# KKKSQJ/DeepLearning

Hardware: AMD Instinct MI355X
Metric: images/sec (higher is better)
Workload: dtype bf16; 1 GPU; model=resnet50, global_batch=256, image_size=224, parallelism=dp1

## Files before the change

### csrc/batchnorm.hip

```cpp
#include "common.h"
#include "vec.h"

namespace dla {

template <typename dev_t>
__global__ void bn_stats_kernel(const dev_t* __restrict__ x, float* __restrict__ sums,
                                int N, int C, int64_t HW) {
  __shared__ float smem[16];
  const int c = blockIdx.x;
  const int64_t total = (int64_t)N * HW;
  float sum = 0.f, sumsq = 0.f;
  for (int64_t m = (int64_t)blockIdx.y * blockDim.x + threadIdx.x; m < total;
       m += (int64_t)gridDim.y * blockDim.x) {
    const int64_t n = m / HW, hw = m % HW;
    const float f = to_f32(x[(n * C + c) * HW + hw]);
    sum += f;
    sumsq += f * f;
  }
  sum = block_reduce_sum(sum, smem);
  sumsq = block_reduce_sum(sumsq, smem);
  if (threadIdx.x == 0) {
    atomicAdd(&sums[c], sum);
    atomicAdd(&sums[C + c], sumsq);
  }
}

__device__ __forceinline__ void bn_finalize_channel(
    int c, float sum, float sumsq, const float* __restrict__ weight,
    const float* __restrict__ bias, float* __restrict__ mean,
    float* __restrict__ rstd, float* __restrict__ running_mean,
    float* __restrict__ running_var, float* __restrict__ scale,
    float* __restrict__ shift, float count, float eps, float momentum) {
  const float mu = sum / count;
  const float var = fmaxf(sumsq / count - mu * mu, 0.f);
  const float rs = rsqrtf(var + eps);
  mean[c] = mu;
  rstd[c] = rs;
  if (running_mean != nullptr && momentum > 0.f) {
    const float unbiased = var * count / fmaxf(count - 1.f, 1.f);
    running_mean[c] = (1.f - momentum) * running_mean[c] + momentum * mu;
    running_var[c] = (1.f - momentum) * running_var[c] + momentum * unbiased;
  }
  const float sc = weight[c] * rs;
  scale[c] = sc;
  shift[c] = bias[c] - mu * sc;
}

__global__ void bn_finalize_kernel(const float* __restrict__ sums,
                                   const float* __restrict__ weight,
                                   const float* __restrict__ bias,
                                   float* __restrict__ mean, float* __restrict__ rstd,
                                   float* __restrict__ running_mean,
                                   float* __restrict__ running_var,
                                   float* __restrict__ scale, float* __restrict__ shift,
                                   int C, float count, float eps, float momentum) {
  const int c = blockIdx.x * blockDim.x + threadIdx.x;
  if (c >= C) return;
  bn_finalize_channel(c, sums[c], sums[C + c], weight, bias, mean, rstd,
                      running_mean, running_var, scale, shift, count, eps,
                      momentum);
}

constexpr int kFinCh = 16, kFinRows = 64;

__global__ void __launch_bounds__(kFinCh * kFinRows)
bn_finalize_parts_kernel(const float* __restrict__ parts, int n_parts,
                         const float* __restrict__ weight,
                         const float* __restrict__ bias,
                         float* __restrict__ mean, float* __restrict__ rstd,
                         float* __restrict__ running_mean,
                         float* __restrict__ running_var,
                         float* __restrict__ scale, float* __restrict__ shift,
                         int C, float count, float eps, float momentum) {
  __shared__ float ls[2][kFinRows][kFinCh + 1];
  const int cl = threadIdx.x % kFinCh, rl = threadIdx.x / kFinCh;
  const int c = blockIdx.x * kFinCh + cl;
  float s = 0.f, q = 0.f;
  if (c < C) {
#pragma unroll 4
    for (int r = rl; r < n_parts; r += kFinRows) {
      const float* p = parts + (int64_t)r * 2 * C;
      s += p[c];
      q += p[C + c];
    }
  }
  ls[0][rl][cl] = s;
  ls[1][rl][cl] = q;
  __syncthreads();
  for (int h = kFinRows / 2; h > 0; h >>= 1) {
    if (rl < h) {
      ls[0][rl][cl] += ls[0][rl + h][cl];
      ls[1][rl][cl] += ls[1][rl + h][cl];
    }
    __syncthreads();
  }
  if (rl == 0 && c < C)
    bn_finalize_channel(c, ls[0][0][cl], ls[1][0][cl], weight, bias, mean,
                        rstd, running_mean, running_var, scale, shift, count,
                        eps, momentum);
}

template <typename dev_t, int V, bool RELU>
__global__ void bn_apply_kernel(const dev_t* __restrict__ x,
                                const float* __restrict__ scale,
                                const float* __restrict__ shift,
                                dev_t* __restrict__ y, int C, int64_t HW,
                                int64_t n_total) {
  const int64_t stride = (int64_t)gridDim.x * blockDim.x * V;
  for (int64_t i = ((int64_t)blockIdx.x * blockDim.x + threadIdx.x) * V;
       i < n_total; i += stride) {
    const int c = (int)((i / HW) % C);
    const float sc = scale[c], sh = shift[c];
    Vec<dev_t, V> xv = vload<dev_t, V>(x + i);
    Vec<dev_t, V> yv;
#pragma unroll
    for (int j = 0; j < V; ++j) {
      float f = to_f32(xv.v[j]) * sc + sh;
      yv.v[j] = from_f32<dev_t>(RELU ? fmaxf(f, 0.f) : f);
    }
    vstore<dev_t, V>(y + i, yv);
  }
}

template <typename dev_t, bool RELU>
__global__ void bn_bwd_stats_kernel(const dev_t* __restrict__ dy,
                                    const dev_t* __restrict__ x,
                                    const dev_t* __restrict__ y,
                                    const float* __restrict__ mean,
                                    const float* __restrict__ rstd,
                                    float* __restrict__ sums,
                                    int N, int C, int64_t HW) {
  __shared__ float smem[16];
  const int c = blockIdx.x;
  const float mu = mean[c], rs = rstd[c];
  const int64_t total = (int64_t)N * HW;
  float s_dy = 0.f, s_dyxh = 0.f;
  for (int64_t m = (int64_t)blockIdx.y * blockDim.x + threadIdx.x; m < total;
       m += (int64_t)gridDim.y * blockDim.x) {
    const int64_t n = m / HW, hw = m % HW;
    const int64_t idx = (n * C + c) * HW + hw;
    float g = to_f32(dy[idx]);
    if (RELU && to_f32(y[idx]) <= 0.f) g = 0.f;
    const float xh = (to_f32(x[idx]) - mu) * rs;
    s_dy += g;
    s_dyxh += g * xh;
  }
  s_dy = block_reduce_sum(s_dy, smem);
  s_dyxh = block_reduce_sum(s_dyxh, smem);
  if (threadIdx.x == 0) {
    atomicAdd(&sums[c], s_dy);
    atomicAdd(&sums[C + c], s_dyxh);
  }
}

template <typename dev_t, bool RELU>
__global__ void bn_bwd_dx_kernel(const dev_t* __restrict__ dy,
                                 const dev_t* __restrict__ x,
                                 const dev_t* __restrict__ y,
                                 const float* __restrict__ mean,
                                 const float* __restrict__ rstd,
                                 const float* __restrict__ weight,
                                 const float* __restrict__ sums,
                                 dev_t* __restrict__ dx, int C, int64_t HW,
                                 int64_t n_total, float inv_count) {
  const int64_t stride = (int64_t)gridDim.x * blockDim.x;
  for (int64_t i = (int64_t)blockIdx.x * blockDim.x + threadIdx.x; i < n_total;
       i += stride) {
    const int c = (int)((i / HW) % C);
    const float mu = mean[c], rs = rstd[c];
    float g = to_f32(dy[i]);
    if (RELU && to_f32(y[i]) <= 0.f) g = 0.f;
    const float xh = (to_f32(x[i]) - mu) * rs;
    const float m_dy = sums[c] * inv_count;
    const float m_dyxh = sums[C + c] * inv_count;
    dx[i] = from_f32<dev_t>(weight[c] * rs * (g - m_dy - xh * m_dyxh));
  }
}



inline int64_t nhwc_used_threads(int lanes_per_row, int64_t rows,
                                 int64_t target_lanes) {
  int64_t k = target_lanes / lanes_per_row;
  if (k > rows) k = rows;
  if (k < 1) k = 1;
  return (int64_t)lanes_per_row * k;
}

template <typename dev_t, int V>
__global__ void bn_stats_nhwc_kernel(const dev_t* __restrict__ x,
                                     float* __restrict__ sums, int C,
                                     int64_t rows, int64_t used) {
  extern __shared__ float ls[];
  for (int i = threadIdx.x; i < 2 * C; i += blockDim.x) ls[i] = 0.f;
  __syncthreads();
  const int64_t t = (int64_t)blockIdx.x * blockDim.x + threadIdx.x;
  const int lanes_per_row = C / V;
  if (t < used) {
    const int c0 = (int)(t % lanes_per_row) * V;
    const int64_t rstride = used / lanes_per_row;
    float s[V], q[V];
#pragma unroll
    for (int j = 0; j < V; ++j) { s[j] = 0.f; q[j] = 0.f; }
    for (int64_t r = t / lanes_per_row; r < rows; r += rstride) {
      Vec<dev_t, V> xv = vload<dev_t, V>(x + r * C + c0);
#pragma unroll
      for (int j = 0; j < V; ++j) {
        const float f = to_f32(xv.v[j]);
        s[j] += f;
        q[j] += f * f;
      }
    }
#pragma unroll
    for (int j = 0; j < V; ++j) {
      atomicAdd(&ls[c0 + j], s[j]);
      atomicAdd(&ls[C + c0 + j], q[j]);
    }
  }
  __syncthreads();
  for (int i = threadIdx.x; i < 2 * C; i += blockDim.x)
    atomicAdd(&sums[i], ls[i]);
}

template <typename dev_t, int V, bool RELU>
__global__ void bn_apply_nhwc_kernel(const dev_t* __restrict__ x,
                                     const float* __restrict__ scale,
                                     const float* __restrict__ shift,
                                     dev_t* __restrict__ y, int C, int64_t rows,
                                     int64_t used) {
  const int64_t t = (int64_t)blockIdx.x * blockDim.x + threadIdx.x;
  if (t >= used) return;
  const int lanes_per_row = C / V;
  const int c0 = (int)(t % lanes_per_row) * V;
  const int64_t rstride = used / lanes_per_row;
  float sc[V], sh[V];
#pragma unroll
  for (int j = 0; j < V; ++j) { sc[j] = scale[c0 + j]; sh[j] = shift[c0 + j]; }
  for (int64_t r = t / lanes_per_row; r < rows; r += rstride) {
    Vec<dev_t, V> xv = vload<dev_t, V>(x + r * C + c0);
    Vec<dev_t, V> yv;
#pragma unroll
    for (int j = 0; j < V; ++j) {
      const float f = to_f32(xv.v[j]) * sc[j] + sh[j];
      yv.v[j] = from_f32<dev_t>(RELU ? fmaxf(f, 0.f) : f);
    }
    vstore<dev_t, V>(y + r * C + c0, yv);
  }
}

template <typename dev_t, int V, bool RELU>
__global__ void bn_bwd_stats_nhwc_kernel(const dev_t* __restrict__ dy,
                                         const dev_t* __restrict__ x,
                                         const dev_t* __restrict__ y,
                                         const float* __restrict__ mean,
                                         const float* __restrict__ rstd,
                                         float* __restrict__ sums, int C,
                                         int64_t rows, int64_t used) {
  extern __shared__ float ls[];
  for (int i = threadIdx.x; i < 2 * C; i += blockDim.x) ls[i] = 0.f;
  __syncthreads();
  const int64_t t = (int64_t)blockIdx.x * blockDim.x + threadIdx.x;
  const int lanes_per_row = C / V;
  if (t < used) {
    const int c0 = (int)(t % lanes_per_row) * V;
    const int64_t rstride = used / lanes_per_row;
    float mu[V], rs[V], s_dy[V], s_dyxh[V];
#pragma unroll
    for (int j = 0; j < V; ++j) {
      mu[j] = mean[c0 + j];
      rs[j] = rstd[c0 + j];
      s_dy[j] = 0.f;
      s_dyxh[j] = 0.f;
    }
    for (int64_t r = t / lanes_per_row; r < rows; r += rstride) {
      const int64_t base = r * C + c0;
      Vec<dev_t, V> dyv = vload<dev_t, V>(dy + base);
      Vec<dev_t, V> xv = vload<dev_t, V>(x + base);
      Vec<dev_t, V> yv;
      if (RELU) yv = vload<dev_t, V>(y + base);
#pragma unroll
      for (int j = 0; j < V; ++j) {
        float g = to_f32(dyv.v[j]);
        if (RELU && to_f32(yv.v[j]) <= 0.f) g = 0.f;
        const float xh = (to_f32(xv.v[j]) - mu[j]) * rs[j];
        s_dy[j] += g;
        s_dyxh[j] += g * xh;
      }
    }
#pragma unroll
    for (int j = 0; j < V; ++j) {
      atomicAdd(&ls[c0 + j], s_dy[j]);
      atomicAdd(&ls[C + c0 + j], s_dyxh[j]);
    }
  }
  __syncthreads();
  for (int i = threadIdx.x; i < 2 * C; i += blockDim.x)
    atomicAdd(&sums[i], ls[i]);
}

template <typename dev_t, int V, bool RELU>
__global__ void bn_bwd_dx_nhwc_kernel(const dev_t* __restrict__ dy,
                                      const dev_t* __restrict__ x,
                                      const dev_t* __restrict__ y,
                                      const float* __restrict__ mean,
                                      const float* __restrict__ rstd,
                                      const float* __restrict__ weight,
                                      const float* __restrict__ sums,
                                      dev_t* __restrict__ dx, int C,
                                      int64_t rows, int64_t used,
                                      float inv_count) {
  const int64_t t = (int64_t)blockIdx.x * blockDim.x + threadIdx.x;
  if (t >= used) return;
  const int lanes_per_row = C / V;
  const int c0 = (int)(t % lanes_per_row) * V;
  const int64_t rstride = used / lanes_per_row;
  float mu[V], rs[V], wr[V], m_dy[V], m_dyxh[V];
#pragma unroll
  for (int j = 0; j < V; ++j) {
    mu[j] = mean[c0 + j];
    rs[j] = rstd[c0 + j];
    wr[j] = weight[c0 + j] * rs[j];
    m_dy[j] = sums[c0 + j] * inv_count;
    m_dyxh[j] = sums[C + c0 + j] * inv_count;
  }
  for (int64_t r = t / lanes_per_row; r < rows; r += rstride) {
    const int64_t base = r * C + c0;
    Vec<dev_t, V> dyv = vload<dev_t, V>(dy + base);
    Vec<dev_t, V> xv = vload<dev_t, V>(x + base);
    Vec<dev_t, V> yv;
    if (RELU) yv = vload<dev_t, V>(y + base);
    Vec<dev_t, V> dxv;
#pragma unroll
    for (int j = 0; j < V; ++j) {
      float g = to_f32(dyv.v[j]);
      if (RELU && to_f32(yv.v[j]) <= 0.f) g = 0.f;
      const float xh = (to_f32(xv.v[j]) - mu[j]) * rs[j];
      dxv.v[j] = from_f32<dev_t>(wr[j] * (g - m_dy[j] - xh * m_dyxh[j]));
    }
    vstore<dev_t, V>(dx + r * C + c0, dxv);
  }
}

template <typename dev_t, int V, bool DUAL>
__global__ void bn_add_relu_nhwc_kernel(const dev_t* __restrict__ x,
                                        const float* __restrict__ scale,
                                        const float* __restrict__ shift,
                                        const dev_t* __restrict__ idn,
                                        const float* __restrict__ scale_d,
                                        const float* __restrict__ shift_d,
                                        dev_t* __restrict__ out, int C,
                                        int64_t rows, int64_t used) {
  const int64_t t = (int64_t)blockIdx.x * blockDim.x + threadIdx.x;
  if (t >= used) return;
  const int lanes_per_row = C / V;
  const int c0 = (int)(t % lanes_per_row) * V;
  const int64_t rstride = used / lanes_per_row;
  float sc[V], sh[V], scd[V];
#pragma unroll
  for (int j = 0; j < V; ++j) {
    sc[j] = scale[c0 + j];
    sh[j] = shift[c0 + j];
    if (DUAL) {
      scd[j] = scale_d[c0 + j];
      sh[j] += shift_d[c0 + j];
    }
  }
  for (int64_t r = t / lanes_per_row; r < rows; r += rstride) {
    const int64_t base = r * C + c0;
    Vec<dev_t, V> xv = vload<dev_t, V>(x + base);
    Vec<dev_t, V> iv = vload<dev_t, V>(idn + base);
    Vec<dev_t, V> ov;
#pragma unroll
    for (int j = 0; j < V; ++j) {
      float f = to_f32(xv.v[j]) * sc[j] + sh[j];
      f += DUAL ? to_f32(iv.v[j]) * scd[j] : to_f32(iv.v[j]);
      ov.v[j] = from_f32<dev_t>(fmaxf(f, 0.f));
    }
    vstore<dev_t, V>(out + base, ov);
  }
}

template <typename dev_t, int V, bool DUAL>
__global__ void bn_join_bwd_stats_nhwc_kernel(
    const dev_t* __restrict__ dy, const dev_t* __restrict__ out,
    const dev_t* __restrict__ x, const float* __restrict__ mean,
    const float* __restrict__ rstd, const dev_t* __restrict__ xd,
    const float* __restrict__ mean_d, const float* __restrict__ rstd_d,
    dev_t* __restrict__ g_out, float* __restrict__ sums, int C, int64_t rows,
    int64_t used) {
  constexpr int NS = DUAL ? 3 : 2;
  extern __shared__ float ls[];
  for (int i = threadIdx.x; i < NS * C; i += blockDim.x) ls[i] = 0.f;
  __syncthreads();
  const int64_t t = (int64_t)blockIdx.x * blockDim.x + threadIdx.x;
  const int lanes_per_row = C / V;
  if (t < used) {
    const int c0 = (int)(t % lanes_per_row) * V;
    const int64_t rstride = used / lanes_per_row;
    float mu[V], rs[V], mud[V], rsd[V], s_g[V], s_gxh[V], s_gxhd[V];
#pragma unroll
    for (int j = 0; j < V; ++j) {
      mu[j] = mean[c0 + j];
      rs[j] = rstd[c0 + j];
      mud[j] = DUAL ? mean_d[c0 + j] : 0.f;
      rsd[j] = DUAL ? rstd_d[c0 + j] : 0.f;
      s_g[j] = 0.f;
      s_gxh[j] = 0.f;
      s_gxhd[j] = 0.f;
    }
    for (int64_t r = t / lanes_per_row; r < rows; r += rstride) {
      const int64_t base = r * C + c0;
      Vec<dev_t, V> dyv = vload<dev_t, V>(dy + base);
      Vec<dev_t, V> ov = vload<dev_t, V>(out + base);
      Vec<dev_t, V> xv = vload<dev_t, V>(x + base);
      Vec<dev_t, V> xdv;
      if (DUAL) xdv = vload<dev_t, V>(xd + base);
      Vec<dev_t, V> gv;
#pragma unroll
      for (int j = 0; j < V; ++j) {
        const bool on = to_f32(ov.v[j]) > 0.f;
        gv.v[j] = on ? dyv.v[j] : from_f32<dev_t>(0.f);
        const float g = on ? to_f32(dyv.v[j]) : 0.f;
        s_g[j] += g;
        s_gxh[j] += g * ((to_f32(xv.v[j]) - mu[j]) * rs[j]);
        if (DUAL) s_gxhd[j] += g * ((to_f32(xdv.v[j]) - mud[j]) * rsd[j]);
      }
      vstore<dev_t, V>(g_out + base, gv);
    }
#pragma unroll
    for (int j = 0; j < V; ++j) {
      atomicAdd(&ls[c0 + j], s_g[j]);
      atomicAdd(&ls[C + c0 + j], s_gxh[j]);
      if (DUAL) atomicAdd(&ls[2 * C + c0 + j], s_gxhd[j]);
    }
  }
  __syncthreads();
  for (int i = threadIdx.x; i < NS * C; i += blockDim.x)
    atomicAdd(&sums[i], ls[i]);
}

template <typename dev_t, int V>
__global__ void bn_join_bwd_dx_dual_nhwc_kernel(
    const dev_t* __restrict__ g, const dev_t* __restrict__ x,
    const dev_t* __restrict__ xd, const float* __restrict__ mean,
    const float* __restrict__ rstd, const float* __restrict__ weight,
    const float* __restrict__ mean_d, const float* __restrict__ rstd_d,
    const float* __restrict__ weight_d, const float* __restrict__ sums,
    dev_t* __restrict__ dx, dev_t* __restrict__ dxd, int C, int64_t rows,
    int64_t used, float inv_count) {
  const int64_t t = (int64_t)blockIdx.x * blockDim.x + threadIdx.x;
  if (t >= used) return;
  const int lanes_per_row = C / V;
  const int c0 = (int)(t % lanes_per_row) * V;
  const int64_t rstride = used / lanes_per_row;
  float mu[V], rs[V], wr[V], mud[V], rsd[V], wrd[V], m_g[V], m_gxh[V],
      m_gxhd[V];
#pragma unroll
  for (int j = 0; j < V; ++j) {
    mu[j] = mean[c0 + j];
    rs[j] = rstd[c0 + j];
    wr[j] = weight[c0 + j] * rs[j];
    mud[j] = mean_d[c0 + j];
    rsd[j] = rstd_d[c0 + j];
    wrd[j] = weight_d[c0 + j] * rsd[j];
    m_g[j] = sums[c0 + j] * inv_count;
    m_gxh[j] = sums[C + c0 + j] * inv_count;
    m_gxhd[j] = sums[2 * C + c0 + j] * inv_count;
  }
  for (int64_t r = t / lanes_per_row; r < rows; r += rstride) {
    const int64_t base = r * C + c0;
    Vec<dev_t, V> gv = vload<dev_t, V>(g + base);
    Vec<dev_t, V> xv = vload<dev_t, V>(x + base);
    Vec<dev_t, V> xdv = vload<dev_t, V>(xd + base);
    Vec<dev_t, V> dxv, dxdv;
#pragma unroll
    for (int j = 0; j < V; ++j) {
      const float gg = to_f32(gv.v[j]) - m_g[j];
      const float xh = (to_f32(xv.v[j]) - mu[j]) * rs[j];
      const float xhd = (to_f32(xdv.v[j]) - mud[j]) * rsd[j];
      dxv.v[j] = from_f32<dev_t>(wr[j] * (gg - xh * m_gxh[j]));
      dxdv.v[j] = from_f32<dev_t>(wrd[j] * (gg - xhd * m_gxhd[j]));
    }
    vstore<dev_t, V>(dx + base, dxv);
    vstore<dev_t, V>(dxd + base, dxdv);
  }
}

inline bool is_nhwc(const torch::Tensor& t) {
  return t.dim() == 4 && t.is_contiguous(at::MemoryFormat::ChannelsLast) &&
         !t.is_contiguous();
}

struct BnFinalized {
  torch::Tensor mean, rstd, scale, shift;
};

inline BnFinalized bn_finalize_launch(
    const torch::Tensor& sums, const torch::Tensor& weight,
    const torch::Tensor& bias, c10::optional<torch::Tensor>& running_mean,
    c10::optional<torch::Tensor>& running_var, int C, int64_t rows,
    double momentum, double eps) {
  TORCH_CHECK(sums.is_cuda() && sums.scalar_type() == torch::kFloat &&
                  sums.is_contiguous(),
              "bn sums must be a contiguous fp32 GPU tensor");
  TORCH_CHECK((sums.dim() == 1 && sums.size(0) == 2 * C) ||
                  (sums.dim() == 2 && sums.size(0) >= 1 &&
                   sums.size(1) == 2 * C),
              "bn sums must be [2C] or [n_parts, 2C]");
  TORCH_CHECK(weight.numel() == C && bias.numel() == C,
              "bn weight/bias must have C elements");
  auto opts_f = sums.options();
  BnFinalized f{torch::empty({C}, opts_f), torch::empty({C}, opts_f),
                torch::empty({C}, opts_f), torch::empty({C}, opts_f)};
  auto w32 = weight.to(torch::kFloat).contiguous();
  auto b32 = bias.to(torch::kFloat).contiguous();
  float* rm = running_mean.has_value() ? running_mean->data_ptr<float>() : nullptr;
  float* rv = running_var.has_value() ? running_var->data_ptr<float>() : nullptr;
  const int n_parts = sums.dim() == 2 ? (int)sums.size(0) : 1;
  if (n_parts > 1) {
    hipLaunchKernelGGL(bn_finalize_parts_kernel, dim3((C + kFinCh - 1) / kFinCh),
                       dim3(kFinCh * kFinRows), 0, stream(),
                       sums.data_ptr<float>(), n_parts, w32.data_ptr<float>(),
                       b32.data_ptr<float>(), f.mean.data_ptr<float>(),
                       f.rstd.data_ptr<float>(), rm, rv,
                       f.scale.data_ptr<float>(), f.shift.data_ptr<float>(), C,
                       (float)rows, (float)eps, (float)momentum);
  } else {
    hipLaunchKernelGGL(bn_finalize_kernel, dim3((C + 255) / 256), dim3(256), 0,
                       stream(), sums.data_ptr<float>(), w32.data_ptr<float>(),
                       b32.data_ptr<float>(), f.mean.data_ptr<float>(),
                       f.rstd.data_ptr<float>(), rm, rv,
                       f.scale.data_ptr<float>(), f.shift.data_ptr<float>(), C,
                       (float)rows, (float)eps, (float)momentum);
  }
  return f;
}

inline torch::Tensor bn_param_grad(const torch::Tensor& sums, int64_t offset,
                                   int C, const torch::Tensor& weight) {
  return sums.narrow(0, offset, C).to(weight.scalar_type());
}

inline bool is_nhwc_rows(const torch::Tensor& t) {
  return t.dim() == 4 && t.is_contiguous(at::MemoryFormat::ChannelsLast);
}

}

std::vector<torch::Tensor> batchnorm_fwd(torch::Tensor x, torch::Tensor weight,
                                         torch::Tensor bias,
                                         c10::optional<torch::Tensor> running_mean,
                                         c10::optional<torch::Tensor> running_var,
                                         double momentum, double eps, bool relu) {
  DLA_CHECK_CUDA(x);
  TORCH_CHECK(x.dim() == 4, "batchnorm_fwd expects a 4D tensor");
  const bool nhwc = dla::is_nhwc(x);
  TORCH_CHECK(nhwc || x.is_contiguous(), "batchnorm_fwd: x must be contiguous "
              "(NCHW or channels_last)");
  const int N = (int)x.size(0), C = (int)x.size(1);
  const int64_t HW = x.size(2) * x.size(3);
  auto opts_f = x.options().dtype(torch::kFloat);
  auto sums = torch::zeros({2 * C}, opts_f);
  auto mean = torch::empty({C}, opts_f);
  auto rstd = torch::empty({C}, opts_f);
  auto scale = torch::empty({C}, opts_f);
  auto shift = torch::empty({C}, opts_f);
  auto y = torch::empty_like(x);
  auto w32 = weight.to(torch::kFloat);
  auto b32 = bias.to(torch::kFloat);

  const int64_t rows = (int64_t)N * HW;
  const int ysplit = (int)std::min<int64_t>((rows + 65535) / 65536 + 1,
                                            std::max(1, 2048 / C));
  DLA_DISPATCH_FLOAT_TYPES(x.scalar_type(), "batchnorm_fwd", [&] {
    if (nhwc) {
      constexpr int VM = 16 / (int)sizeof(dev_t);
      auto stats = [&](auto vtag) {
        constexpr int V = decltype(vtag)::value;
        const int lanes = C / V;
        const int64_t used = dla::nhwc_used_threads(lanes, rows, 262144);
        const int lds = 2 * C * sizeof(float);
        hipLaunchKernelGGL((dla::bn_stats_nhwc_kernel<dev_t, V>),
                           dim3((int)((used + 255) / 256)), dim3(256), lds,
                           dla::stream(), (const dev_t*)x.data_ptr(),
                           sums.data_ptr<float>(), C, rows, used);
      };
      if (C % VM == 0) stats(std::integral_constant<int, VM>{});
      else if (C % 2 == 0) stats(std::integral_constant<int, 2>{});
      else stats(std::integral_constant<int, 1>{});
    } else {
      hipLaunchKernelGGL((dla::bn_stats_kernel<dev_t>), dim3(C, ysplit), dim3(256), 0,
                         dla::stream(), (const dev_t*)x.data_ptr(),
                         sums.data_ptr<float>(), N, C, HW);
    }
    hipLaunchKernelGGL(dla::bn_finalize_kernel, dim3((C + 255) / 256), dim3(256), 0,
                       dla::stream(), sums.data_ptr<float>(), w32.data_ptr<float>(),
                       b32.data_ptr<float>(), mean.data_ptr<float>(),
                       rstd.data_ptr<float>(),
                       running_mean.has_value() ? running_mean->data_ptr<float>() : nullptr,
                       running_var.has_value() ? running_var->data_ptr<float>() : nullptr,
                       scale.data_ptr<float>(), shift.data_ptr<float>(), C,
                       (float)rows, (float)eps, (float)momentum);
    const int64_t n_total = x.numel();
    constexpr int VMAX = 16 / (int)sizeof(dev_t);
    auto launch = [&](auto vtag, auto rtag) {
      constexpr int V = decltype(vtag)::value;
      constexpr bool R = decltype(rtag)::value;
      if (nhwc) {
        const int lanes = C / V;
        const int64_t used = dla::nhwc_used_threads(lanes, rows, 524288);
        hipLaunchKernelGGL((dla::bn_apply_nhwc_kernel<dev_t, V, R>),
                           dim3((int)((used + 255) / 256)), dim3(256), 0,
                           dla::stream(), (const dev_t*)x.data_ptr(),
                           scale.data_ptr<float>(), shift.data_ptr<float>(),
                           (dev_t*)y.data_ptr(), C, rows, used);
        return;
      }
      const int grid = dla::grid_1d((n_total + V - 1) / V, 256);
      if (false) ;
      else
        hipLaunchKernelGGL((dla::bn_apply_kernel<dev_t, V, R>), dim3(grid), dim3(256),
                           0, dla::stream(), (const dev_t*)x.data_ptr(),
                           scale.data_ptr<float>(), shift.data_ptr<float>(),
                           (dev_t*)y.data_ptr(), C, HW, n_total);
    };
    const bool vec_ok = nhwc ? (C % VMAX == 0) : (HW % VMAX == 0);
    if (vec_ok) {
      if (relu) launch(std::integral_constant<int, VMAX>{}, std::true_type{});
      else launch(std::integral_constant<int, VMAX>{}, std::false_type{});
    } else {
      if (relu) launch(std::integral_constant<int, 1>{}, std::true_type{});
      else launch(std::integral_constant<int, 1>{}, std::false_type{});
    }
  });
  HIP_CHECK_ERR();
  return {y, mean, rstd};
}

std::vector<torch::Tensor> batchnorm_fwd_from_sums(
    torch::Tensor x, torch::Tensor weight, torch::Tensor bias,
    torch::Tensor sums, c10::optional<torch::Tensor> running_mean,
    c10::optional<torch::Tensor> running_var, double momentum, double eps,
    bool relu) {
  DLA_CHECK_CUDA(x);
  TORCH_CHECK(x.dim() == 4, "batchnorm_fwd_from_sums expects a 4D tensor");
  const bool nhwc = dla::is_nhwc(x);
  TORCH_CHECK(nhwc || x.is_contiguous(),
              "batchnorm_fwd_from_sums: x must be contiguous");
  const int N = (int)x.size(0), C = (int)x.size(1);
  const int64_t HW = x.size(2) * x.size(3);
  auto y = torch::empty_like(x);
  const int64_t rows = (int64_t)N * HW;
  auto fin = dla::bn_finalize_launch(sums, weight, bias, running_mean,
                                     running_var, C, rows, momentum, eps);
  auto& mean = fin.mean;
  auto& rstd = fin.rstd;
  auto& scale = fin.scale;
  auto& shift = fin.shift;
  DLA_DISPATCH_FLOAT_TYPES(x.scalar_type(), "batchnorm_fwd_from_sums", [&] {
    const int64_t n_total = x.numel();
    constexpr int VMAX = 16 / (int)sizeof(dev_t);
    auto launch = [&](auto vtag, auto rtag) {
      constexpr int V = decltype(vtag)::value;
      constexpr bool R = decltype(rtag)::value;
      if (nhwc) {
        const int lanes = C / V;
        const int64_t used = dla::nhwc_used_threads(lanes, rows, 524288);
        hipLaunchKernelGGL((dla::bn_apply_nhwc_kernel<dev_t, V, R>),
                           dim3((int)((used + 255) / 256)), dim3(256), 0,
                           dla::stream(), (const dev_t*)x.data_ptr(),
                           scale.data_ptr<float>(), shift.data_ptr<float>(),
                           (dev_t*)y.data_ptr(), C, rows, used);
        return;
      }
      const int grid = dla::grid_1d((n_total + V - 1) / V, 256);
      hipLaunchKernelGGL((dla::bn_apply_kernel<dev_t, V, R>), dim3(grid),
                         dim3(256), 0, dla::stream(),
                         (const dev_t*)x.data_ptr(), scale.data_ptr<float>(),
                         shift.data_ptr<float>(), (dev_t*)y.data_ptr(), C, HW,
                         n_total);
    };
    const bool vec_ok = nhwc ? (C % VMAX == 0) : (HW % VMAX == 0);
    if (vec_ok) {
      if (relu) launch(std::integral_constant<int, VMAX>{}, std::true_type{});
      else launch(std::integral_constant<int, VMAX>{}, std::false_type{});
    } else {
      if (relu) launch(std::integral_constant<int, 1>{}, std::true_type{});
      else launch(std::integral_constant<int, 1>{}, std::false_type{});
    }
  });
  HIP_CHECK_ERR();
  return {y, mean, rstd};
}

torch::Tensor bn_apply(torch::Tensor x, torch::Tensor scale, torch::Tensor shift,
                       bool relu) {
  DLA_CHECK_CUDA(x);
  TORCH_CHECK(x.dim() == 4, "bn_apply expects a 4D tensor");
  const bool nhwc = dla::is_nhwc(x);
  TORCH_CHECK(nhwc || x.is_contiguous(), "bn_apply: x must be contiguous");
  const int C = (int)x.size(1);
  const int64_t HW = x.size(2) * x.size(3);
  auto y = torch::empty_like(x);
  auto sc = scale.to(torch::kFloat).contiguous();
  auto sh = shift.to(torch::kFloat).contiguous();
  const int64_t n_total = x.numel();
  DLA_DISPATCH_FLOAT_TYPES(x.scalar_type(), "bn_apply", [&] {
    constexpr int VMAX = 16 / (int)sizeof(dev_t);
    auto launch = [&](auto vtag, auto rtag) {
      constexpr int V = decltype(vtag)::value;
      constexpr bool R = decltype(rtag)::value;
      if (nhwc) {
        const int64_t rows = n_total / C;
        const int lanes = C / V;
        const int64_t used = dla::nhwc_used_threads(lanes, rows, 524288);
        hipLaunchKernelGGL((dla::bn_apply_nhwc_kernel<dev_t, V, R>),
                           dim3((int)((used + 255) / 256)), dim3(256), 0,
                           dla::stream(), (const dev_t*)x.data_ptr(),
                           sc.data_ptr<float>(), sh.data_ptr<float>(),
                           (dev_t*)y.data_ptr(), C, rows, used);
        return;
      }
      const int grid = dla::grid_1d((n_total + V - 1) / V, 256);
      if (false) ;
      else
        hipLaunchKernelGGL((dla::bn_apply_kernel<dev_t, V, R>), dim3(grid), dim3(256),
                           0, dla::stream(), (const dev_t*)x.data_ptr(),
                           sc.data_ptr<float>(), sh.data_ptr<float>(),
                           (dev_t*)y.data_ptr(), C, HW, n_total);
    };
    const bool vec_ok = nhwc ? (C % VMAX == 0) : (HW % VMAX == 0);
    if (vec_ok) {
      if (relu) launch(std::integral_constant<int, VMAX>{}, std::true_type{});
      else launch(std::integral_constant<int, VMAX>{}, std::false_type{});
    } else {
      if (relu) launch(std::integral_constant<int, 1>{}, std::true_type{});
      else launch(std::integral_constant<int, 1>{}, std::false_type{});
    }
  });
  HIP_CHECK_ERR();
  return y;
}

std::vector<torch::Tensor> batchnorm_bwd(torch::Tensor dy, torch::Tensor x,
                                         c10::optional<torch::Tensor> y,
                                         torch::Tensor weight, torch::Tensor mean,
                                         torch::Tensor rstd, bool relu) {
  DLA_CHECK_CUDA(dy); DLA_CHECK_CUDA(x);
  const bool nhwc = dla::is_nhwc(x);
  TORCH_CHECK(nhwc || x.is_contiguous(), "batchnorm_bwd: x must be contiguous");
  if (nhwc && !dla::is_nhwc(dy)) dy = dy.contiguous(at::MemoryFormat::ChannelsLast);
  if (!nhwc) dy = dy.contiguous();
  const int N = (int)x.size(0), C = (int)x.size(1);
  const int64_t HW = x.size(2) * x.size(3);
  const int64_t rows = (int64_t)N * HW;
  auto opts_f = x.options().dtype(torch::kFloat);
  auto sums = torch::zeros({2 * C}, opts_f);
  auto dx = torch::empty_like(x);
  auto w32 = weight.to(torch::kFloat);
  const int ysplit = (int)std::min<int64_t>((rows + 65535) / 65536 + 1,
                                            std::max(1, 2048 / C));
  TORCH_CHECK(!relu || y.has_value(), "batchnorm_bwd: relu mask needs y");
  DLA_DISPATCH_FLOAT_TYPES(x.scalar_type(), "batchnorm_bwd", [&] {
    const dev_t* yp = y.has_value() ? (const dev_t*)y->data_ptr() : nullptr;
    auto launch_stats = [&](auto rtag) {
      constexpr bool R = decltype(rtag)::value;
      if (nhwc) {
        constexpr int VM = 16 / (int)sizeof(dev_t);
        auto stats = [&](auto vtag) {
          constexpr int V = decltype(vtag)::value;
          const int lanes = C / V;
          const int64_t used = dla::nhwc_used_threads(lanes, rows, 262144);
          const int lds = 2 * C * sizeof(float);
          hipLaunchKernelGGL((dla::bn_bwd_stats_nhwc_kernel<dev_t, V, R>),
                             dim3((int)((used + 255) / 256)), dim3(256), lds,
                             dla::stream(), (const dev_t*)dy.data_ptr(),
                             (const dev_t*)x.data_ptr(), yp, mean.data_ptr<float>(),
                             rstd.data_ptr<float>(), sums.data_ptr<float>(), C,
                             rows, used);
        };
        if (C % VM == 0) stats(std::integral_constant<int, VM>{});
        else if (C % 2 == 0) stats(std::integral_constant<int, 2>{});
        else stats(std::integral_constant<int, 1>{});
      } else {
        hipLaunchKernelGGL((dla::bn_bwd_stats_kernel<dev_t, R>), dim3(C, ysplit),
                           dim3(256), 0, dla::stream(), (const dev_t*)dy.data_ptr(),
                           (const dev_t*)x.data_ptr(), yp, mean.data_ptr<float>(),
                           rstd.data_ptr<float>(), sums.data_ptr<float>(), N, C, HW);
      }
    };
    if (relu) launch_stats(std::true_type{});
    else launch_stats(std::false_type{});

    const int64_t n_total = x.numel();
    const float inv_count = 1.f / (float)rows;
    constexpr int VMAX = 16 / (int)sizeof(dev_t);
    auto launch_dx = [&](auto vtag, auto rtag) {
      constexpr int V = decltype(vtag)::value;
      constexpr bool R = decltype(rtag)::value;
      if (nhwc) {
        const int lanes = C / V;
        const int64_t used = dla::nhwc_used_threads(lanes, rows, 524288);
        hipLaunchKernelGGL((dla::bn_bwd_dx_nhwc_kernel<dev_t, V, R>),
                           dim3((int)((used + 255) / 256)), dim3(256), 0,
                           dla::stream(), (const dev_t*)dy.data_ptr(),
                           (const dev_t*)x.data_ptr(), yp, mean.data_ptr<float>(),
                           rstd.data_ptr<float>(), w32.data_ptr<float>(),
                           sums.data_ptr<float>(), (dev_t*)dx.data_ptr(), C,
                           rows, used, inv_count);
      } else {
        hipLaunchKernelGGL((dla::bn_bwd_dx_kernel<dev_t, R>), dim3(dla::grid_1d(n_total, 256)),
                           dim3(256), 0, dla::stream(), (const dev_t*)dy.data_ptr(),
                           (const dev_t*)x.data_ptr(), yp, mean.data_ptr<float>(),
                           rstd.data_ptr<float>(), w32.data_ptr<float>(),
                           sums.data_ptr<float>(), (dev_t*)dx.data_ptr(), C, HW,
                           n_total, inv_count);
      }
    };
    const bool vec_ok = nhwc && (C % VMAX == 0);
    if (vec_ok) {
      if (relu) launch_dx(std::integral_constant<int, VMAX>{}, std::true_type{});
      else launch_dx(std::integral_constant<int, VMAX>{}, std::false_type{});
    } else {
      if (relu) launch_dx(std::integral_constant<int, 1>{}, std::true_type{});
      else launch_dx(std::integral_constant<int, 1>{}, std::false_type{});
    }
  });
  HIP_CHECK_ERR();
  return {dx, dla::bn_param_grad(sums, C, C, weight),
          dla::bn_param_grad(sums, 0, C, weight)};
}

namespace dla {

inline void join_check(const torch::Tensor& x, const torch::Tensor& other,
                       const char* what) {
  TORCH_CHECK(other.is_cuda() && other.scalar_type() == x.scalar_type() &&
                  other.sizes() == x.sizes() && is_nhwc_rows(other),
              "bn join: ", what, " must match x (shape, dtype, channels_last)");
}

inline int join_vec(const torch::Tensor& x) {
  const int vmax = 16 / (int)x.element_size();
  TORCH_CHECK(x.size(1) % vmax == 0,
              "bn join: C must be a multiple of ", vmax);
  return vmax;
}

}

std::vector<torch::Tensor> bn_add_relu_fwd_from_sums(
    torch::Tensor x, torch::Tensor weight, torch::Tensor bias,
    torch::Tensor sums, c10::optional<torch::Tensor> running_mean,
    c10::optional<torch::Tensor> running_var, double momentum, double eps,
    torch::Tensor identity) {
  DLA_CHECK_CUDA(x);
  TORCH_CHECK(dla::is_nhwc_rows(x), "bn_add_relu: x must be channels_last");
  dla::join_check(x, identity, "identity");
  dla::join_vec(x);
  const int C = (int)x.size(1);
  const int64_t rows = x.numel() / C;
  auto fin = dla::bn_finalize_launch(sums, weight, bias, running_mean,
                                     running_var, C, rows, momentum, eps);
  auto out = torch::empty_like(x);
  DLA_DISPATCH_FLOAT_TYPES(x.scalar_type(), "bn_add_relu_fwd_from_sums", [&] {
    constexpr int V = 16 / (int)sizeof(dev_t);
    const int64_t used = dla::nhwc_used_threads(C / V, rows, 524288);
    hipLaunchKernelGGL((dla::bn_add_relu_nhwc_kernel<dev_t, V, false>),
                       dim3((int)((used + 255) / 256)), dim3(256), 0,
                       dla::stream(), (const dev_t*)x.data_ptr(),
                       fin.scale.data_ptr<float>(), fin.shift.data_ptr<float>(),
                       (const dev_t*)identity.data_ptr(), nullptr, nullptr,
                       (dev_t*)out.data_ptr(), C, rows, used);
  });
  HIP_CHECK_ERR();
  return {out, fin.mean, fin.rstd};
}

std::vector<torch::Tensor> bn_add_relu_dual_fwd_from_sums(
    torch::Tensor x, torch::Tensor weight, torch::Tensor bias,
    torch::Tensor sums, c10::optional<torch::Tensor> running_mean,
    c10::optional<torch::Tensor> running_var, double momentum, double eps,
    torch::Tensor xd, torch::Tensor weight_d, torch::Tensor bias_d,
    torch::Tensor sums_d, c10::optional<torch::Tensor> running_mean_d,
    c10::optional<torch::Tensor> running_var_d, double momentum_d,
    double eps_d) {
  DLA_CHECK_CUDA(x);
  TORCH_CHECK(dla::is_nhwc_rows(x), "bn_add_relu_dual: x must be channels_last");
  dla::join_check(x, xd, "xd");
  dla::join_vec(x);
  const int C = (int)x.size(1);
  const int64_t rows = x.numel() / C;
  auto fin = dla::bn_finalize_launch(sums, weight, bias, running_mean,
                                     running_var, C, rows, momentum, eps);
  auto fd = dla::bn_finalize_launch(sums_d, weight_d, bias_d, running_mean_d,
                                    running_var_d, C, rows, momentum_d, eps_d);
  auto out = torch::empty_like(x);
  DLA_DISPATCH_FLOAT_TYPES(x.scalar_type(), "bn_add_relu_dual_fwd_from_sums", [&] {
    constexpr int V = 16 / (int)sizeof(dev_t);
    const int64_t used = dla::nhwc_used_threads(C / V, rows, 524288);
    hipLaunchKernelGGL((dla::bn_add_relu_nhwc_kernel<dev_t, V, true>),
                       dim3((int)((used + 255) / 256)), dim3(256), 0,
                       dla::stream(), (const dev_t*)x.data_ptr(),
                       fin.scale.data_ptr<float>(), fin.shift.data_ptr<float>(),
                       (const dev_t*)xd.data_ptr(), fd.scale.data_ptr<float>(),
                       fd.shift.data_ptr<float>(), (dev_t*)out.data_ptr(), C,
                       rows, used);
  });
  HIP_CHECK_ERR();
  return {out, fin.mean, fin.rstd, fd.mean, fd.rstd};
}

std::vector<torch::Tensor> bn_add_relu_bwd(torch::Tensor dy, torch::Tensor out,
                                           torch::Tensor x, torch::Tensor weight,
                                           torch::Tensor mean,
                                           torch::Tensor rstd) {
  DLA_CHECK_CUDA(x);
  TORCH_CHECK(dla::is_nhwc_rows(x), "bn_add_relu_bwd: x must be channels_last");
  dla::join_check(x, out, "out");
  if (!dla::is_nhwc_rows(dy)) dy = dy.contiguous(at::MemoryFormat::ChannelsLast);
  dla::join_check(x, dy, "dy");
  dla::join_vec(x);
  const int C = (int)x.size(1);
  const int64_t rows = x.numel() / C;
  TORCH_CHECK(mean.numel() == C && rstd.numel() == C && weight.numel() == C,
              "bn_add_relu_bwd: per-channel tensors must have C elements");
  auto sums = torch::zeros({2 * C}, x.options().dtype(torch::kFloat));
  auto g = torch::empty_like(x);
  auto dx = torch::empty_like(x);
  auto w32 = weight.to(torch::kFloat).contiguous();
  DLA_DISPATCH_FLOAT_TYPES(x.scalar_type(), "bn_add_relu_bwd", [&] {
    constexpr int V = 16 / (int)sizeof(dev_t);
    const int lanes = C / V;
    const int64_t used_s = dla::nhwc_used_threads(lanes, rows, 262144);
    hipLaunchKernelGGL((dla::bn_join_bwd_stats_nhwc_kernel<dev_t, V, false>),
                       dim3((int)((used_s + 255) / 256)), dim3(256),
                       2 * C * sizeof(float), dla::stream(),
                       (const dev_t*)dy.data_ptr(), (const dev_t*)out.data_ptr(),
                       (const dev_t*)x.data_ptr(), mean.data_ptr<float>(),
                       rstd.data_ptr<float>(), nullptr, nullptr, nullptr,
                       (dev_t*)g.data_ptr(), sums.data_ptr<float>(), C, rows,
                       used_s);
    const int64_t used = dla::nhwc_used_threads(lanes, rows, 524288);
    hipLaunchKernelGGL((dla::bn_bwd_dx_nhwc_kernel<dev_t, V, false>),
                       dim3((int)((used + 255) / 256)), dim3(256), 0,
                       dla::stream(), (const dev_t*)g.data_ptr(),
                       (const dev_t*)x.data_ptr(), nullptr,
                       mean.data_ptr<float>(), rstd.data_ptr<float>(),
                       w32.data_ptr<float>(), sums.data_ptr<float>(),
                       (dev_t*)dx.data_ptr(), C, rows, used,
                       1.f / (float)rows);
  });
  HIP_CHECK_ERR();
  return {g, dx, dla::bn_param_grad(sums, C, C, weight),
          dla::bn_param_grad(sums, 0, C, weight)};
}

std::vector<torch::Tensor> bn_add_relu_dual_bwd(
    torch::Tensor dy, torch::Tensor out, torch::Tensor x, torch::Tensor weight,
    torch::Tensor mean, torch::Tensor rstd, torch::Tensor xd,
    torch::Tensor weight_d, torch::Tensor mean_d, torch::Tensor rstd_d) {
  DLA_CHECK_CUDA(x);
  TORCH_CHECK(dla::is_nhwc_rows(x), "bn_add_relu_dual_bwd: x must be channels_last");
  dla::join_check(x, out, "out");
  dla::join_check(x, xd, "xd");
  if (!dla::is_nhwc_rows(dy)) dy = dy.contiguous(at::MemoryFormat::ChannelsLast);
  dla::join_check(x, dy, "dy");
  dla::join_vec(x);
  const int C = (int)x.size(1);
  const int64_t rows = x.numel() / C;
  TORCH_CHECK(mean.numel() == C && rstd.numel() == C && weight.numel() == C &&
                  mean_d.numel() == C && rstd_d.numel() == C &&
                  weight_d.numel() == C,
              "bn_add_relu_dual_bwd: per-channel tensors must have C elements");
  auto sums = torch::zeros({3 * C}, x.options().dtype(torch::kFloat));
  auto g = torch::empty_like(x);
  auto dx = torch::empty_like(x);
  auto dxd = torch::empty_like(x);
  auto w32 = weight.to(torch::kFloat).contiguous();
  auto wd32 = weight_d.to(torch::kFloat).contiguous();
  DLA_DISPATCH_FLOAT_TYPES(x.scalar_type(), "bn_add_relu_dual_bwd", [&] {
    constexpr int V = 16 / (int)sizeof(dev_t);
    const int lanes = C / V;
    const int64_t used_s = dla::nhwc_used_threads(lanes, rows, 262144);
    hipLaunchKernelGGL((dla::bn_join_bwd_stats_nhwc_kernel<dev_t, V, true>),
                       dim3((int)((used_s + 255) / 256)), dim3(256),
                       3 * C * sizeof(float), dla::stream(),
                       (const dev_t*)dy.data_ptr(), (const dev_t*)out.data_ptr(),
                       (const dev_t*)x.data_ptr(), mean.data_ptr<float>(),
                       rstd.data_ptr<float>(), (const dev_t*)xd.data_ptr(),
                       mean_d.data_ptr<float>(), rstd_d.data_ptr<float>(),
                       (dev_t*)g.data_ptr(), sums.data_ptr<float>(), C, rows,
                       used_s);
    const int64_t used = dla::nhwc_used_threads(lanes, rows, 524288);
    hipLaunchKernelGGL((dla::bn_join_bwd_dx_dual_nhwc_kernel<dev_t, V>),
                       dim3((int)((used + 255) / 256)), dim3(256), 0,
                       dla::stream(), (const dev_t*)g.data_ptr(),
                       (const dev_t*)x.data_ptr(), (const dev_t*)xd.data_ptr(),
                       mean.data_ptr<float>(), rstd.data_ptr<float>(),
                       w32.data_ptr<float>(), mean_d.data_ptr<float>(),
                       rstd_d.data_ptr<float>(), wd32.data_ptr<float>(),
                       sums.data_ptr<float>(), (dev_t*)dx.data_ptr(),
                       (dev_t*)dxd.data_ptr(), C, rows, used,
                       1.f / (float)rows);
  });
  HIP_CHECK_ERR();
  auto dbias = dla::bn_param_grad(sums, 0, C, weight);
  return {dx, dxd, dla::bn_param_grad(sums, C, C, weight), dbias,
          dla::bn_param_grad(sums, 2 * C, C, weight_d),
          dbias.to(weight_d.scalar_type()).clone()};
}
```

### csrc/bindings.cpp

```cpp
#include <torch/extension.h>

std::vector<torch::Tensor> layernorm_fwd(torch::Tensor x, torch::Tensor w,
                                         torch::Tensor b, double eps);
std::vector<torch::Tensor> layernorm_bwd(torch::Tensor dy, torch::Tensor x,
                                         torch::Tensor w, torch::Tensor mean,
                                         torch::Tensor rstd);
torch::Tensor gelu_fwd(torch::Tensor x);
torch::Tensor gelu_bwd(torch::Tensor dy, torch::Tensor x);
torch::Tensor silu_fwd(torch::Tensor x);
torch::Tensor silu_bwd(torch::Tensor dy, torch::Tensor x);
torch::Tensor add_relu_fwd(torch::Tensor a, torch::Tensor b);
torch::Tensor relu_mask_bwd(torch::Tensor dy, torch::Tensor y);
std::vector<torch::Tensor> batchnorm_fwd(torch::Tensor x, torch::Tensor weight,
                                         torch::Tensor bias,
                                         c10::optional<torch::Tensor> running_mean,
                                         c10::optional<torch::Tensor> running_var,
                                         double momentum, double eps, bool relu);
torch::Tensor bn_apply(torch::Tensor x, torch::Tensor scale, torch::Tensor shift,
                       bool relu);
std::vector<torch::Tensor> batchnorm_bwd(torch::Tensor dy, torch::Tensor x,
                                         c10::optional<torch::Tensor> y,
                                         torch::Tensor weight, torch::Tensor mean,
                                         torch::Tensor rstd, bool relu);
std::vector<torch::Tensor> batchnorm_fwd_from_sums(
    torch::Tensor x, torch::Tensor weight, torch::Tensor bias,
    torch::Tensor sums, c10::optional<torch::Tensor> running_mean,
    c10::optional<torch::Tensor> running_var, double momentum, double eps,
    bool relu);
std::vector<torch::Tensor> bn_add_relu_fwd_from_sums(
    torch::Tensor x, torch::Tensor weight, torch::Tensor bias,
    torch::Tensor sums, c10::optional<torch::Tensor> running_mean,
    c10::optional<torch::Tensor> running_var, double momentum, double eps,
    torch::Tensor identity);
std::vector<torch::Tensor> bn_add_relu_dual_fwd_from_sums(
    torch::Tensor x, torch::Tensor weight, torch::Tensor bias,
    torch::Tensor sums, c10::optional<torch::Tensor> running_mean,
    c10::optional<torch::Tensor> running_var, double momentum, double eps,
    torch::Tensor xd, torch::Tensor weight_d, torch::Tensor bias_d,
    torch::Tensor sums_d, c10::optional<torch::Tensor> running_mean_d,
    c10::optional<torch::Tensor> running_var_d, double momentum_d,
    double eps_d);
std::vector<torch::Tensor> bn_add_relu_bwd(torch::Tensor dy, torch::Tensor out,
                                           torch::Tensor x, torch::Tensor weight,
                                           torch::Tensor mean,
                                           torch::Tensor rstd);
std::vector<torch::Tensor> bn_add_relu_dual_bwd(
    torch::Tensor dy, torch::Tensor out, torch::Tensor x, torch::Tensor weight,
    torch::Tensor mean, torch::Tensor rstd, torch::Tensor xd,
    torch::Tensor weight_d, torch::Tensor mean_d, torch::Tensor rstd_d);
std::vector<torch::Tensor> conv1x1_fwd(torch::Tensor a, torch::Tensor b,
                                       c10::optional<torch::Tensor> bias,
                                       c10::optional<torch::Tensor> scale,
                                       c10::optional<torch::Tensor> shift,
                                       c10::optional<torch::Tensor> residual,
                                       bool relu, bool want_stats);
torch::Tensor conv1x1_wgrad(torch::Tensor dy, torch::Tensor x);
std::vector<torch::Tensor> conv3x3_fwd(torch::Tensor a, torch::Tensor w9,
                                       int64_t imgH, int64_t imgW,
                                       c10::optional<torch::Tensor> bias,
                                       c10::optional<torch::Tensor> scale,
                                       c10::optional<torch::Tensor> shift,
                                       c10::optional<torch::Tensor> residual,
                                       bool relu, bool want_stats);
torch::Tensor conv3x3_wgrad(torch::Tensor dy, torch::Tensor x, int64_t imgH,
                            int64_t imgW);
torch::Tensor transpose2d(torch::Tensor src);
torch::Tensor stride2_gather(torch::Tensor x);
torch::Tensor stride2_scatter(torch::Tensor dy, int64_t IH, int64_t IW);
std::vector<torch::Tensor> softmax_ce_fwd(torch::Tensor logits,
                                          c10::optional<torch::Tensor> target,
                                          c10::optional<torch::Tensor> soft_target,
                                          double smoothing, int64_t ignore_index);
torch::Tensor softmax_ce_bwd(torch::Tensor logits,
                             c10::optional<torch::Tensor> target,
                             c10::optional<torch::Tensor> soft_target,
                             torch::Tensor lse, double smoothing,
                             int64_t ignore_index, torch::Tensor grad_out,
                             torch::Tensor stats);
torch::Tensor focal_loss_fwd(torch::Tensor logits, torch::Tensor targets,
                             double alpha, double gamma);
torch::Tensor focal_loss_bwd(torch::Tensor dloss, torch::Tensor logits,
                             torch::Tensor targets, double alpha, double gamma);
torch::Tensor box_iou_gpu(torch::Tensor a, torch::Tensor b, bool giou);
torch::Tensor nms_gpu(torch::Tensor boxes_sorted, double iou_threshold);
torch::Tensor roialign_fwd(torch::Tensor input, torch::Tensor rois, int64_t PH,
                           int64_t PW, double spatial_scale,
                           int64_t sampling_ratio, bool aligned);
torch::Tensor roialign_bwd(torch::Tensor grad_out, torch::Tensor rois, int64_t N,
                           int64_t C, int64_t H, int64_t W, double spatial_scale,
                           int64_t sampling_ratio, bool aligned);
std::vector<torch::Tensor> attn_fwd(torch::Tensor qkv, int64_t num_heads,
                                    double scale,
                                    c10::optional<torch::Tensor> bias,
                                    c10::optional<torch::Tensor> mask,
                                    bool save_p, bool save_stats);
std::vector<torch::Tensor> attn_bwd(torch::Tensor qkv, torch::Tensor dout,
                                    torch::Tensor stats, torch::Tensor drow,
                                    int64_t num_heads, double scale);
std::vector<torch::Tensor> attn_fwd_cosine(torch::Tensor qkv, int64_t num_heads,
                              torch::Tensor logit_scale,
                              c10::optional<torch::Tensor> bias,
                              c10::optional<torch::Tensor> mask, bool save_p);
torch::Tensor mfma_probe(torch::Tensor A, torch::Tensor B);
torch::Tensor my_add(torch::Tensor a, torch::Tensor b);
std::vector<torch::Tensor> cocoeval_match_image(
    torch::Tensor det_boxes, torch::Tensor det_scores, torch::Tensor gt_boxes,
    torch::Tensor gt_crowd, torch::Tensor iou_thrs, int64_t max_dets,
    c10::optional<torch::Tensor> gt_extra_ignore);
torch::Tensor window_partition_fwd(torch::Tensor x, int64_t ws, int64_t shift);
torch::Tensor window_partition_bwd(torch::Tensor grad, int64_t B, int64_t H,
                                   int64_t W, int64_t ws, int64_t shift);
torch::Tensor window_merge_fwd(torch::Tensor windows, int64_t B, int64_t H,
                               int64_t W, int64_t ws, int64_t shift);
torch::Tensor window_merge_bwd(torch::Tensor grad, int64_t ws, int64_t shift);

PYBIND11_MODULE(TORCH_EXTENSION_NAME, m) {
  m.doc() = "deeplearning_amd gfx950 HIP kernels";
  m.def("layernorm_fwd", &layernorm_fwd);
  m.def("layernorm_bwd", &layernorm_bwd);
  m.def("gelu_fwd", &gelu_fwd);
  m.def("gelu_bwd", &gelu_bwd);
  m.def("silu_fwd", &silu_fwd);
  m.def("silu_bwd", &silu_bwd);
  m.def("add_relu_fwd", &add_relu_fwd);
  m.def("relu_mask_bwd", &relu_mask_bwd);
  m.def("batchnorm_fwd", &batchnorm_fwd);
  m.def("batchnorm_fwd_from_sums", &batchnorm_fwd_from_sums);
  m.def("bn_apply", &bn_apply);
  m.def("batchnorm_bwd", &batchnorm_bwd);
  m.def("bn_add_relu_fwd_from_sums", &bn_add_relu_fwd_from_sums);
  m.def("bn_add_relu_dual_fwd_from_sums", &bn_add_relu_dual_fwd_from_sums);
  m.def("bn_add_relu_bwd", &bn_add_relu_bwd);
  m.def("bn_add_relu_dual_bwd", &bn_add_relu_dual_bwd);
  m.def("conv1x1_fwd", &conv1x1_fwd, py::arg("a"), py::arg("b"),
        py::arg("bias") = py::none(), py::arg("scale") = py::none(),
        py::arg("shift") = py::none(), py::arg("residual") = py::none(),
        py::arg("relu") = false, py::arg("want_stats") = false);
  m.def("conv1x1_wgrad", &conv1x1_wgrad);
  m.def("conv3x3_fwd", &conv3x3_fwd, py::arg("a"), py::arg("w9"),
        py::arg("imgH"), py::arg("imgW"), py::arg("bias") = py::none(),
        py::arg("scale") = py::none(), py::arg("shift") = py::none(),
        py::arg("residual") = py::none(), py::arg("relu") = false,
        py::arg("want_stats") = false);
  m.def("conv3x3_wgrad", &conv3x3_wgrad);
  m.def("transpose2d", &transpose2d);
  m.def("stride2_gather", &stride2_gather);
  m.def("stride2_scatter", &stride2_scatter);
  m.def("softmax_ce_fwd", &softmax_ce_fwd);
  m.def("softmax_ce_bwd", &softmax_ce_bwd);
  m.def("focal_loss_fwd", &focal_loss_fwd);
  m.def("focal_loss_bwd", &focal_loss_bwd);
  m.def("box_iou", &box_iou_gpu);
  m.def("nms", &nms_gpu);
  m.def("roialign_fwd", &roialign_fwd);
  m.def("roialign_bwd", &roialign_bwd);
  m.def("attn_fwd", &attn_fwd, py::arg("qkv"), py::arg("num_heads"),
        py::arg("scale"), py::arg("bias") = py::none(),
        py::arg("mask") = py::none(), py::arg("save_p") = false,
        py::arg("save_stats") = false);
  m.def("attn_bwd", &attn_bwd);
  m.def("attn_fwd_cosine", &attn_fwd_cosine, py::arg("qkv"),
        py::arg("num_heads"), py::arg("logit_scale"),
        py::arg("bias") = py::none(), py::arg("mask") = py::none(),
        py::arg("save_p") = false);
  m.def("mfma_probe", &mfma_probe);
  m.def("cocoeval_match_image", &cocoeval_match_image, py::arg("det_boxes"),
        py::arg("det_scores"), py::arg("gt_boxes"), py::arg("gt_crowd"),
        py::arg("iou_thrs"), py::arg("max_dets"),
        py::arg("gt_extra_ignore") = py::none());
  m.def("my_add", &my_add);
  m.def("window_partition_fwd", &window_partition_fwd);
  m.def("window_partition_bwd", &window_partition_bwd);
  m.def("window_merge_fwd", &window_merge_fwd);
  m.def("window_merge_bwd", &window_merge_bwd);
}
```

### deeplearning_amd/models/classification/resnet.py

```python
from __future__ import annotations

import torch
import torch.nn as nn

from ...ops import BatchNorm2d, add_relu
from ...ops.conv1x1 import (can_pass_input, conv1x1_bn, conv_bn,
                            conv_bn_add_relu)
from ..registry import register_model


def _downsample_fwd(downsample, x):
    if (isinstance(downsample, nn.Sequential) and len(downsample) == 2 and
            isinstance(downsample[0], nn.Conv2d)):
        return conv_bn(x, downsample[0], downsample[1])
    return downsample(x)


class _NormRelu(nn.Sequential):

    def __init__(self, norm, c):
        super().__init__(norm(c), nn.ReLU(inplace=True))


def make_norm(norm_layer, c, relu=False):
    if not relu:
        return norm_layer(c)
    try:
        return norm_layer(c, relu=True)
    except TypeError:
        return _NormRelu(norm_layer, c)


def conv3x3(cin, cout, stride=1, groups=1, dilation=1):
    return nn.Conv2d(cin, cout, 3, stride=stride, padding=dilation, groups=groups,
                     bias=False, dilation=dilation)


def conv1x1(cin, cout, stride=1):
    return nn.Conv2d(cin, cout, 1, stride=stride, bias=False)


class BasicBlock(nn.Module):
    expansion = 1

    def __init__(self, inplanes, planes, stride=1, downsample=None, groups=1,
                 base_width=64, dilation=1, norm_layer=None):
        super().__init__()
        norm_layer = norm_layer or BatchNorm2d
        if groups != 1 or base_width != 64:
            raise ValueError("BasicBlock only supports groups=1, base_width=64")
        self.conv1 = conv3x3(inplanes, planes, stride)
        self.bn1 = make_norm(norm_layer, planes, relu=True)
        self.conv2 = conv3x3(planes, planes)
        self.bn2 = norm_layer(planes)
        self.downsample = downsample
        self.stride = stride

    def forward(self, x):
        identity = x
        out = conv_bn(x, self.conv1, self.bn1)
        out = conv_bn(out, self.conv2, self.bn2)
        if self.downsample is not None:
            identity = _downsample_fwd(self.downsample, x)
        return add_relu(out, identity)


class Bottleneck(nn.Module):
    expansion = 4

    def __init__(self, inplanes, planes, stride=1, downsample=None, groups=1,
                 base_width=64, dilation=1, norm_layer=None):
        super().__init__()
        norm_layer = norm_layer or BatchNorm2d
        width = int(planes * (base_width / 64.0)) * groups
        self.conv1 = conv1x1(inplanes, width)
        self.bn1 = make_norm(norm_layer, width, relu=True)
        self.conv2 = conv3x3(width, width, stride, groups, dilation)
        self.bn2 = make_norm(norm_layer, width, relu=True)
        self.conv3 = conv1x1(width, planes * self.expansion)
        self.bn3 = norm_layer(planes * self.expansion)
        self.downsample = downsample
        self.stride = stride

    def forward(self, x):
        identity = x
        if self.downsample is None and can_pass_input(x, self.conv1, self.bn1):
            out, identity = conv1x1_bn(x, self.conv1, self.bn1,
                                       pass_input=True)
        else:
            out = conv_bn(x, self.conv1, self.bn1)
        out = conv_bn(out, self.conv2, self.bn2)
        return conv_bn_add_relu(out, self.conv3, self.bn3, identity=identity,
                                x_down=x, downsample=self.downsample)


class ResNet(nn.Module):
    def __init__(self, block, layers, num_classes=1000, groups=1, width_per_group=64,
                 replace_stride_with_dilation=None, norm_layer=None,
                 zero_init_residual=False, include_top=True):
        super().__init__()
        self._norm_layer = norm_layer or BatchNorm2d
        self.inplanes = 64
        self.dilation = 1
        replace_stride_with_dilation = replace_stride_with_dilation or [False] * 3
        self.groups = groups
        self.base_width = width_per_group
        self.include_top = include_top

        self.conv1 = nn.Conv2d(3, 64, 7, stride=2, padding=3, bias=False)
        self.bn1 = make_norm(self._norm_layer, 64, relu=True)
        self.maxpool = nn.MaxPool2d(3, stride=2, padding=1)
        self.layer1 = self._make_layer(block, 64, layers[0])
        self.layer2 = self._make_layer(block, 128, layers[1], stride=2,
                                       dilate=replace_stride_with_dilation[0])
        self.layer3 = self._make_layer(block, 256, layers[2], stride=2,
                                       dilate=replace_stride_with_dilation[1])
        self.layer4 = self._make_layer(block, 512, layers[3], stride=2,
                                       dilate=replace_stride_with_dilation[2])
        if include_top:
            self.avgpool = nn.AdaptiveAvgPool2d(1)
            self.fc = nn.Linear(512 * block.expansion, num_classes)

        for m in self.modules():
            if isinstance(m, nn.Conv2d):
                nn.init.kaiming_normal_(m.weight, mode="fan_out", nonlinearity="relu")
            elif isinstance(m, (nn.BatchNorm2d, nn.GroupNorm)):
                nn.init.ones_(m.weight)
                nn.init.zeros_(m.bias)
        if zero_init_residual:
            for m in self.modules():
                if isinstance(m, Bottleneck):
                    nn.init.zeros_(m.bn3.weight)
                elif isinstance(m, BasicBlock):
                    nn.init.zeros_(m.bn2.weight)

    def _make_layer(self, block, planes, blocks, stride=1, dilate=False):
        norm_layer = self._norm_layer
        downsample = None
        prev_dilation = self.dilation
        if dilate:
            self.dilation *= stride
            stride = 1
        if stride != 1 or self.inplanes != planes * block.expansion:
            downsample = nn.Sequential(
                conv1x1(self.inplanes, planes * block.expansion, stride),
                norm_layer(planes * block.expansion),
            )
        layers = [block(self.inplanes, planes, stride, downsample, self.groups,
                        self.base_width, prev_dilation, norm_layer)]
        self.inplanes = planes * block.expansion
        for _ in range(1, blocks):
            layers.append(block(self.inplanes, planes, groups=self.groups,
                                base_width=self.base_width, dilation=self.dilation,
                                norm_layer=norm_layer))
        return nn.Sequential(*layers)

    def forward_features(self, x):
        x = self.maxpool(self.bn1(self.conv1(x)))
        x = self.layer1(x)
        x = self.layer2(x)
        x = self.layer3(x)
        x = self.layer4(x)
        return x

    def forward(self, x):
        x = self.forward_features(x)
        if self.include_top:
            x = self.avgpool(x)
            x = torch.flatten(x, 1)
            x = self.fc(x)
        return x


@register_model
def resnet18(num_classes=1000, **kw):
    return ResNet(BasicBlock, [2, 2, 2, 2], num_classes=num_classes, **kw)


@register_model
def resnet34(num_classes=1000, **kw):
    return ResNet(BasicBlock, [3, 4, 6, 3], num_classes=num_classes, **kw)


@register_model
def resnet50(num_classes=1000, **kw):
    return ResNet(Bottleneck, [3, 4, 6, 3], num_classes=num_classes, **kw)


@register_model
def resnet101(num_classes=1000, **kw):
    return ResNet(Bottleneck, [3, 4, 23, 3], num_classes=num_classes, **kw)


@register_model
def resnet152(num_classes=1000, **kw):
    return ResNet(Bottleneck, [3, 8, 36, 3], num_classes=num_classes, **kw)


@register_model
def resnext50_32x4d(num_classes=1000, **kw):
    return ResNet(Bottleneck, [3, 4, 6, 3], num_classes=num_classes, groups=32,
                  width_per_group=4, **kw)


@register_model
def resnext101_32x8d(num_classes=1000, **kw):
    return ResNet(Bottleneck, [3, 4, 23, 3], num_classes=num_classes, groups=32,
                  width_per_group=8, **kw)


@register_model
def wide_resnet50_2(num_classes=1000, **kw):
    return ResNet(Bottleneck, [3, 4, 6, 3], num_classes=num_classes,
                  width_per_group=128, **kw)


@register_model
def wide_resnet101_2(num_classes=1000, **kw):
    return ResNet(Bottleneck, [3, 4, 23, 3], num_classes=num_classes,
                  width_per_group=128, **kw)
```

### deeplearning_amd/ops/__init__.py

```python
from ._ext import ext, has_ext, use_hip
from .activations import GELU, SiLU, add_relu, gelu, silu
from .batchnorm import BatchNorm2d, FrozenBatchNorm2d
from .conv1x1 import conv1x1_bn, conv_bn, conv_bn_add_relu
from .boxes import (batched_nms, bbox_iou_aligned, box_area, box_iou,
                    clip_boxes_to_image, generalized_box_iou, nms,
                    remove_small_boxes)
from .drop import DropPath, drop_path
from .ema import ModelEMA
from .layernorm import LayerNorm, LayerNorm2d, layer_norm
from .losses import (CrossEntropyLoss, cross_entropy, sigmoid_focal_loss,
                     soft_target_cross_entropy)
from .roi_align import MultiScaleRoIAlign, roi_align
from .window import (roll_and_window_partition, window_merge_and_roll,
                     window_partition_eager, window_reverse_eager)

__all__ = [
    "ext", "has_ext", "use_hip",
    "gelu", "silu", "add_relu", "GELU", "SiLU",
    "BatchNorm2d", "FrozenBatchNorm2d",
    "conv_bn", "conv1x1_bn", "conv_bn_add_relu",
    "box_iou", "generalized_box_iou", "bbox_iou_aligned", "box_area", "nms",
    "batched_nms", "clip_boxes_to_image", "remove_small_boxes",
    "DropPath", "drop_path", "ModelEMA",
    "LayerNorm", "LayerNorm2d", "layer_norm",
    "CrossEntropyLoss", "cross_entropy", "soft_target_cross_entropy",
    "sigmoid_focal_loss",
    "MultiScaleRoIAlign", "roi_align",
    "roll_and_window_partition", "window_merge_and_roll",
    "window_partition_eager", "window_reverse_eager",
]
```

### deeplearning_amd/ops/batchnorm.py

```python
from __future__ import annotations

import torch
import torch.nn as nn
import torch.nn.functional as F

from ._ext import dense, ext, use_hip


class _BNFn(torch.autograd.Function):
    @staticmethod
    def forward(ctx, x, weight, bias, running_mean, running_var, momentum, eps, relu):
        x = dense(x)
        y, mean, rstd = ext().batchnorm_fwd(
            x, weight, bias, running_mean, running_var, momentum, eps, relu)
        ctx.save_for_backward(x, y, weight, mean, rstd)
        ctx.relu = relu
        return y

    @staticmethod
    def backward(ctx, dy):
        x, y, weight, mean, rstd = ctx.saved_tensors
        dx, dw, db = ext().batchnorm_bwd(
            dy, x, y if ctx.relu else None, weight, mean, rstd, ctx.relu)
        return dx, dw, db, None, None, None, None, None


class BatchNorm2d(nn.BatchNorm2d):

    def __init__(self, num_features, eps=1e-5, momentum=0.1, relu=False):
        super().__init__(num_features, eps=eps, momentum=momentum, affine=True,
                         track_running_stats=True)
        self.relu = relu

    def _eaf(self) -> float:
        if self.momentum is not None:
            return self.momentum
        if self.training and self.num_batches_tracked is not None:
            return 1.0 / float(max(int(self.num_batches_tracked), 1))
        return 0.0

    def forward(self, x):
        if not use_hip(x):
            if self.training and self.momentum is None and \
                    self.num_batches_tracked is not None:
                self.num_batches_tracked.add_(1)
            y = F.batch_norm(x, self.running_mean, self.running_var, self.weight,
                             self.bias, self.training, self._eaf(), self.eps)
            return torch.relu(y) if self.relu else y
        if self.running_mean.dtype != torch.float32:
            self.running_mean.data = self.running_mean.data.float()
            self.running_var.data = self.running_var.data.float()
        if self.training:
            if self.num_batches_tracked is not None:
                self.num_batches_tracked.add_(1)
            return _BNFn.apply(x, self.weight, self.bias, self.running_mean,
                               self.running_var, self._eaf(), self.eps,
                               self.relu)
        rstd = torch.rsqrt(self.running_var.float() + self.eps)
        scale = self.weight.float() * rstd
        shift = self.bias.float() - self.running_mean.float() * scale
        if torch.is_grad_enabled() and (x.requires_grad or self.weight.requires_grad):
            y = x * scale.reshape(1, -1, 1, 1).to(x.dtype) + shift.reshape(1, -1, 1, 1).to(x.dtype)
            return torch.relu(y) if self.relu else y
        return ext().bn_apply(dense(x), scale, shift, self.relu)


class FrozenBatchNorm2d(nn.Module):

    def __init__(self, num_features, eps=1e-5):
        super().__init__()
        self.eps = eps
        self.register_buffer("weight", torch.ones(num_features))
        self.register_buffer("bias", torch.zeros(num_features))
        self.register_buffer("running_mean", torch.zeros(num_features))
        self.register_buffer("running_var", torch.ones(num_features))

    def _load_from_state_dict(self, state_dict, prefix, *args, **kwargs):
        state_dict.pop(prefix + "num_batches_tracked", None)
        super()._load_from_state_dict(state_dict, prefix, *args, **kwargs)

    def forward(self, x):
        rstd = torch.rsqrt(self.running_var.float() + self.eps)
        scale = self.weight.float() * rstd
        shift = self.bias.float() - self.running_mean.float() * scale
        if use_hip(x) and not (torch.is_grad_enabled() and x.requires_grad):
            return ext().bn_apply(dense(x), scale, shift, False)
        sc = scale.reshape(1, -1, 1, 1).to(x.dtype)
        sh = shift.reshape(1, -1, 1, 1).to(x.dtype)
        return x * sc + sh
```

### deeplearning_amd/ops/conv1x1.py

```python
from __future__ import annotations

import os

import torch
import torch.nn.functional as F
from torch import nn

from ._ext import ext, use_hip


def _flatten_nhwc(x: torch.Tensor) -> torch.Tensor:
    B, C, H, W = x.shape
    return x.permute(0, 2, 3, 1).reshape(B * H * W, C)


def _unflatten_nhwc(y2d: torch.Tensor, B: int, H: int, W: int) -> torch.Tensor:
    return y2d.view(B, H, W, -1).permute(0, 3, 1, 2)


class _Conv1x1Fn(torch.autograd.Function):

    @staticmethod
    def forward(ctx, x2d, w, bias, scale, shift, residual, relu, want_stats,
                pass_input=False):
        xb = x2d if x2d.dtype == torch.bfloat16 else x2d.to(torch.bfloat16)
        wb = w if w.dtype == torch.bfloat16 else w.to(torch.bfloat16)
        wb = wb.contiguous()
        y2d, sums = ext().conv1x1_fwd(xb, wb, bias, scale, shift, residual,
                                      relu, want_stats)
        ctx.save_for_backward(xb, wb)
        ctx.x_dtype = x2d.dtype
        ctx.w_dtype = w.dtype
        ctx.pass_input = pass_input
        outs = (y2d,)
        if want_stats:
            ctx.mark_non_differentiable(sums)
            outs += (sums,)
        if pass_input:
            ctx.set_materialize_grads(False)
            outs += (x2d,)
        return outs if len(outs) > 1 else y2d

    @staticmethod
    def backward(ctx, dy2d, *rest):
        xb, wb = ctx.saved_tensors
        d_alias = rest[-1] if ctx.pass_input else None
        if d_alias is not None:
            d_alias = d_alias.contiguous()
        dx = dw = db = None
        if dy2d is None:
            if d_alias is not None and ctx.needs_input_grad[0]:
                dx = d_alias.to(ctx.x_dtype)
            return dx, None, None, None, None, None, None, None, None
        dy2d = dy2d.contiguous()
        if dy2d.dtype != torch.bfloat16:
            dy2d = dy2d.to(torch.bfloat16)
        if ctx.needs_input_grad[0]:
            wt = ext().transpose2d(wb)
            if d_alias is not None and d_alias.dtype != torch.bfloat16:
                d_alias = d_alias.to(torch.bfloat16)
            dx, _ = ext().conv1x1_fwd(dy2d, wt, None, None, None, d_alias,
                                      False, False)
            if dx.dtype != ctx.x_dtype:
                dx = dx.to(ctx.x_dtype)
        if ctx.needs_input_grad[1]:
            dw = ext().conv1x1_wgrad(dy2d, xb)
            if dw.dtype != ctx.w_dtype:
                dw = dw.to(ctx.w_dtype)
        if ctx.needs_input_grad[2]:
            db = dy2d.float().sum(0)
        return dx, dw, db, None, None, None, None, None, None


class _BNFromStatsFn(torch.autograd.Function):

    @staticmethod
    def forward(ctx, x, weight, bias, sums, running_mean, running_var,
                momentum, eps, relu):
        y, mean, rstd = ext().batchnorm_fwd_from_sums(
            x, weight, bias, sums, running_mean, running_var, momentum, eps,
            relu)
        ctx.save_for_backward(x, y, weight, mean, rstd)
        ctx.relu = relu
        return y

    @staticmethod
    def backward(ctx, dy):
        x, y, weight, mean, rstd = ctx.saved_tensors
        dx, dw, db = ext().batchnorm_bwd(
            dy, x, y if ctx.relu else None, weight, mean, rstd, ctx.relu)
        return dx, dw, db, None, None, None, None, None, None


class _Stride2Fn(torch.autograd.Function):

    @staticmethod
    def forward(ctx, x):
        ctx.ihw = (x.shape[2], x.shape[3])
        return ext().stride2_gather(x)

    @staticmethod
    def backward(ctx, dy):
        if not dy.is_contiguous(memory_format=torch.channels_last):
            dy = dy.contiguous(memory_format=torch.channels_last)
        return ext().stride2_scatter(dy, *ctx.ihw)


def _conv1x1_disabled() -> bool:
    return os.environ.get("DLA_NO_CONV1X1", "0") == "1"


def can_fuse_conv1x1(x: torch.Tensor, conv: nn.Conv2d) -> bool:
    if _conv1x1_disabled() or not use_hip(x):
        return False
    if x.dtype != torch.bfloat16:
        return False
    if conv.kernel_size != (1, 1) or conv.groups != 1:
        return False
    if conv.padding != (0, 0) or conv.dilation != (1, 1):
        return False
    if conv.stride not in ((1, 1), (2, 2)):
        return False
    cin, cout = conv.in_channels, conv.out_channels
    if cin % 64 != 0 or cout % 64 != 0:
        return False
    return x.dim() == 4 and x.is_contiguous(memory_format=torch.channels_last)


def _prep(x: torch.Tensor, conv: nn.Conv2d):
    stride = conv.stride[0]
    if stride == 2:
        x = _Stride2Fn.apply(x)
    B, C, H, W = x.shape
    x2d = _flatten_nhwc(x)
    w2d = conv.weight.reshape(conv.weight.shape[0], conv.weight.shape[1])
    bias = conv.bias.float() if conv.bias is not None else None
    return x2d, w2d, bias, (B, H, W)


def conv1x1(x: torch.Tensor, conv: nn.Conv2d) -> torch.Tensor:
    x2d, wb, bias, (B, H, W) = _prep(x, conv)
    y2d = _Conv1x1Fn.apply(x2d, wb, bias, None, None, None, False, False)
    return _unflatten_nhwc(y2d, B, H, W)


def _fp32_running_stats(bn) -> None:
    if bn.running_mean.dtype != torch.float32:
        bn.running_mean.data = bn.running_mean.data.float()
        bn.running_var.data = bn.running_var.data.float()


def _conv1x1_train_stats(x: torch.Tensor, conv: nn.Conv2d, bn,
                         pass_input: bool = False):
    x2d, wb, bias, (B, H, W) = _prep(x, conv)
    _fp32_running_stats(bn)
    if bn.num_batches_tracked is not None:
        bn.num_batches_tracked.add_(1)
    momentum = bn._eaf() if hasattr(bn, "_eaf") else (bn.momentum or 0.0)
    outs = _Conv1x1Fn.apply(x2d, wb, bias, None, None, None, False, True,
                            pass_input)
    alias = _unflatten_nhwc(outs[2], B, H, W) if pass_input else None
    return _unflatten_nhwc(outs[0], B, H, W), outs[1], momentum, alias


def conv1x1_bn(x: torch.Tensor, conv: nn.Conv2d, bn,
               pass_input: bool = False):
    relu = bool(getattr(bn, "relu", False))
    if bn.training:
        y_raw, partials, momentum, alias = _conv1x1_train_stats(
            x, conv, bn, pass_input)
        y = _BNFromStatsFn.apply(y_raw, bn.weight, bn.bias, partials,
                                 bn.running_mean, bn.running_var, momentum,
                                 bn.eps, relu)
        return (y, alias) if pass_input else y
    if pass_input:
        raise ValueError("conv1x1_bn: pass_input needs train mode")

    x2d, wb, bias, (B, H, W) = _prep(x, conv)
    _fp32_running_stats(bn)

    if not bn.training:
        rstd = torch.rsqrt(bn.running_var + bn.eps)
        scale = bn.weight.float() * rstd
        shift = bn.bias.float() - bn.running_mean * scale
        if not (torch.is_grad_enabled() and
                (x.requires_grad or conv.weight.requires_grad or
                 bn.weight.requires_grad)):
            y2d, _ = ext().conv1x1_fwd(
                x2d.to(torch.bfloat16), wb.to(torch.bfloat16).contiguous(),
                bias, scale.contiguous(), shift.contiguous(), None, relu,
                False)
            return _unflatten_nhwc(y2d, B, H, W)
        y2d = _Conv1x1Fn.apply(x2d, wb, bias, None, None, None, False, False)
        y = _unflatten_nhwc(y2d, B, H, W)
        y = y * scale.reshape(1, -1, 1, 1).to(y.dtype) + \
            shift.reshape(1, -1, 1, 1).to(y.dtype)
        return torch.relu(y) if relu else y


class _BNJoinFn(torch.autograd.Function):

    @staticmethod
    def forward(ctx, x_raw, weight, bias, partials, running_mean,
                running_var, momentum, eps, identity):
        out, mean, rstd = ext().bn_add_relu_fwd_from_sums(
            x_raw, weight, bias, partials, running_mean, running_var,
            momentum, eps, identity)
        ctx.save_for_backward(x_raw, out, weight, mean, rstd)
        return out

    @staticmethod
    def backward(ctx, dy):
        x_raw, out, weight, mean, rstd = ctx.saved_tensors
        g, dx, dw, db = ext().bn_add_relu_bwd(dy, out, x_raw, weight, mean,
                                              rstd)
        return dx, dw, db, None, None, None, None, None, g


class _BNJoinDualFn(torch.autograd.Function):

    @staticmethod
    def forward(ctx, x_raw, weight, bias, partials, running_mean,
                running_var, momentum, eps, xd_raw, weight_d, bias_d,
                partials_d, running_mean_d, running_var_d, momentum_d, eps_d):
        out, mean, rstd, mean_d, rstd_d = \
            ext().bn_add_relu_dual_fwd_from_sums(
                x_raw, weight, bias, partials, running_mean, running_var,
                momentum, eps, xd_raw, weight_d, bias_d, partials_d,
                running_mean_d, running_var_d, momentum_d, eps_d)
        ctx.save_for_backward(x_raw, xd_raw, out, weight, mean, rstd,
                              weight_d, mean_d, rstd_d)
        return out

    @staticmethod
    def backward(ctx, dy):
        (x_raw, xd_raw, out, weight, mean, rstd, weight_d, mean_d,
         rstd_d) = ctx.saved_tensors
        dx, dxd, dw, db, dwd, dbd = ext().bn_add_relu_dual_bwd(
            dy, out, x_raw, weight, mean, rstd, xd_raw, weight_d, mean_d,
            rstd_d)
        return (dx, dw, db, None, None, None, None, None,
                dxd, dwd, dbd, None, None, None, None, None)


def _fused_join_disabled() -> bool:
    return os.environ.get("DLA_NO_FUSED_JOIN", "0") == "1"


def _join_bn_ok(conv: nn.Conv2d, bn) -> bool:
    from .batchnorm import BatchNorm2d

    return (type(bn) is BatchNorm2d and bn.training and
            not getattr(bn, "relu", False) and conv.bias is None)


def can_pass_input(x: torch.Tensor, conv: nn.Conv2d, bn) -> bool:
    from .batchnorm import BatchNorm2d

    return (not _fused_join_disabled() and can_fuse_conv1x1(x, conv) and
            conv.stride == (1, 1) and type(bn) is BatchNorm2d and
            bn.training and torch.is_grad_enabled() and x.requires_grad)


def can_fuse_join(x: torch.Tensor, conv: nn.Conv2d, bn, identity=None,
                  x_down=None, downsample=None) -> bool:
    if _fused_join_disabled() or not can_fuse_conv1x1(x, conv) or \
            not _join_bn_ok(conv, bn):
        return False
    if downsample is not None:
        if not (isinstance(downsample, nn.Sequential) and
                len(downsample) == 2 and
                isinstance(downsample[0], nn.Conv2d)):
            return False
        return (x_down is not None and
                can_fuse_conv1x1(x_down, downsample[0]) and
                _join_bn_ok(downsample[0], downsample[1]) and
                downsample[0].out_channels == conv.out_channels)
    return (identity is not None and use_hip(identity) and
            identity.dtype == torch.bfloat16 and identity.dim() == 4 and
            identity.is_contiguous(memory_format=torch.channels_last))


def conv_bn_add_relu(x: torch.Tensor, conv: nn.Conv2d, bn, identity=None,
                     x_down=None, downsample=None) -> torch.Tensor:
    if can_fuse_join(x, conv, bn, identity, x_down, downsample):
        y_raw, partials, momentum, _ = _conv1x1_train_stats(x, conv, bn)
        if downsample is None:
            if identity.shape != y_raw.shape:
                raise ValueError("conv_bn_add_relu: identity shape mismatch")
            return _BNJoinFn.apply(y_raw, bn.weight, bn.bias, partials,
                                   bn.running_mean, bn.running_var, momentum,
                                   bn.eps, identity)
        conv_d, bn_d = downsample[0], downsample[1]
        yd_raw, partials_d, momentum_d, _ = _conv1x1_train_stats(
            x_down, conv_d, bn_d)
        if yd_raw.shape != y_raw.shape:
            raise ValueError("conv_bn_add_relu: downsample shape mismatch")
        return _BNJoinDualFn.apply(
            y_raw, bn.weight, bn.bias, partials, bn.running_mean,
            bn.running_var, momentum, bn.eps, yd_raw, bn_d.weight, bn_d.bias,
            partials_d, bn_d.running_mean, bn_d.running_var, momentum_d,
            bn_d.eps)
    from .activations import add_relu

    out = conv_bn(x, conv, bn)
    if downsample is not None:
        if (isinstance(downsample, nn.Sequential) and len(downsample) == 2
                and isinstance(downsample[0], nn.Conv2d)):
            identity = conv_bn(x_down, downsample[0], downsample[1])
        else:
            identity = downsample(x_down)
    return add_relu(out, identity)


def conv_bn(x: torch.Tensor, conv: nn.Conv2d, bn) -> torch.Tensor:
    from .batchnorm import BatchNorm2d

    if isinstance(bn, BatchNorm2d):
        if can_fuse_conv1x1(x, conv):
            return conv1x1_bn(x, conv, bn)
        if can_fuse_conv3x3(x, conv):
            return conv3x3_bn(x, conv, bn)
    return bn(conv(x))


class _Conv3x3Fn(torch.autograd.Function):

    @staticmethod
    def forward(ctx, x4d, w, want_stats):
        B, C, H, W = x4d.shape
        xb = x4d if x4d.dtype == torch.bfloat16 else x4d.to(torch.bfloat16)
        wb = w if w.dtype == torch.bfloat16 else w.to(torch.bfloat16)
        a = _flatten_nhwc(xb)
        w9 = wb.permute(0, 2, 3, 1).reshape(w.shape[0], -1).contiguous()
        y2d, sums = ext().conv3x3_fwd(a, w9, H, W, None, None, None, None,
                                      False, want_stats)
        ctx.save_for_backward(xb, wb)
        ctx.w_dtype = w.dtype
        ctx.x_dtype = x4d.dtype
        y = _unflatten_nhwc(y2d, B, H, W)
        if want_stats:
            ctx.mark_non_differentiable(sums)
            return y, sums
        return y

    @staticmethod
    def backward(ctx, dy, *unused):
        xb, wb = ctx.saved_tensors
        B, C, H, W = xb.shape
        if not dy.is_contiguous(memory_format=torch.channels_last):
            dy = dy.contiguous(memory_format=torch.channels_last)
        if dy.dtype != torch.bfloat16:
            dy = dy.to(torch.bfloat16)
        dy2d = _flatten_nhwc(dy)
        dx = dw = None
        if ctx.needs_input_grad[0]:
            wd = wb.flip(2, 3).transpose(0, 1)
            wd9 = wd.permute(0, 2, 3, 1).reshape(C, -1).contiguous()
            dx2d, _ = ext().conv3x3_fwd(dy2d, wd9, H, W, None, None, None,
                                        None, False, False)
            dx = _unflatten_nhwc(dx2d, B, H, W)
            if dx.dtype != ctx.x_dtype:
                dx = dx.to(ctx.x_dtype)
        if ctx.needs_input_grad[1]:
            dw9 = ext().conv3x3_wgrad(dy2d, _flatten_nhwc(xb), H, W)
            dw = dw9.view(wb.shape[0], 3, 3, C).permute(0, 3, 1, 2)
            if dw.dtype != ctx.w_dtype:
                dw = dw.to(ctx.w_dtype)
            else:
                dw = dw.contiguous()
        return dx, dw, None


def _conv3x3_enabled() -> bool:
    return os.environ.get("DLA_CONV3X3", "0") == "1"


def can_fuse_conv3x3(x: torch.Tensor, conv: nn.Conv2d) -> bool:
    if _conv1x1_disabled() or not _conv3x3_enabled() or not use_hip(x):
        return False
    if x.dtype != torch.bfloat16:
        return False
    if conv.kernel_size != (3, 3) or conv.groups != 1:
        return False
    if conv.padding != (1, 1) or conv.dilation != (1, 1) or \
            conv.stride != (1, 1) or conv.bias is not None:
        return False
    if conv.in_channels % 64 != 0 or conv.out_channels % 64 != 0:
        return False
    return x.dim() == 4 and x.is_contiguous(memory_format=torch.channels_last)


def conv3x3_bn(x: torch.Tensor, conv: nn.Conv2d, bn) -> torch.Tensor:
    relu = bool(getattr(bn, "relu", False))
    B, C, H, W = x.shape
    if bn.running_mean.dtype != torch.float32:
        bn.running_mean.data = bn.running_mean.data.float()
        bn.running_var.data = bn.running_var.data.float()
    if not bn.training:
        rstd = torch.rsqrt(bn.running_var + bn.eps)
        scale = bn.weight.float() * rstd
        shift = bn.bias.float() - bn.running_mean * scale
        if not (torch.is_grad_enabled() and
                (x.requires_grad or conv.weight.requires_grad or
                 bn.weight.requires_grad)):
            xb = x.to(torch.bfloat16)
            wb = conv.weight.to(torch.bfloat16)
            w9 = wb.permute(0, 2, 3, 1).reshape(wb.shape[0], -1).contiguous()
            y2d, _ = ext().conv3x3_fwd(_flatten_nhwc(xb), w9, H, W, None,
                                       scale.contiguous(), shift.contiguous(),
                                       None, relu, False)
            return _unflatten_nhwc(y2d, B, H, W)
        y = _Conv3x3Fn.apply(x, conv.weight, False)
        y = y * scale.reshape(1, -1, 1, 1).to(y.dtype) + \
            shift.reshape(1, -1, 1, 1).to(y.dtype)
        return torch.relu(y) if relu else y
    if bn.num_batches_tracked is not None:
        bn.num_batches_tracked.add_(1)
    momentum = bn._eaf() if hasattr(bn, "_eaf") else (bn.momentum or 0.0)
    y_raw, partials = _Conv3x3Fn.apply(x, conv.weight, True)
    return _BNFromStatsFn.apply(y_raw, bn.weight, bn.bias, partials,
                                bn.running_mean, bn.running_var, momentum,
                                bn.eps, relu)
```

Before: 8120 images/s.

## Fuse stem BN+ReLU+maxpool and recompute ReLU mask from x in BN backward

Adds a fused channels_last kernel that applies BN, ReLU and 3x3/s2 maxpool in one pass. It stores a uint8 argmax slot per output, so the full-resolution BN output of the stem is never written or saved. The fused backward routes gradients through the slots and BN. Separately, BN-with-ReLU backward now rebuilds the ReLU mask from x using the forward's scale/shift instead of loading the saved y, which saves memory and one tensor read per element. The cost is a few extra FMAs, a new code path with tie-breaking that may differ slightly from PyTorch's maxpool, and more template variants.

```diff
diff --git a/csrc/batchnorm.hip b/csrc/batchnorm.hip
--- a/csrc/batchnorm.hip
+++ b/csrc/batchnorm.hip
@@ -2,6 +2,10 @@
 #include "vec.h"
 
 namespace dla {
+
+__device__ __forceinline__ float bn_pre(float x, float sc, float sh) {
+  return fmaf(x, sc, sh);
+}
 
 template <typename dev_t>
 __global__ void bn_stats_kernel(const dev_t* __restrict__ x, float* __restrict__ sums,
@@ -115,7 +119,7 @@
     Vec<dev_t, V> yv;
 #pragma unroll
     for (int j = 0; j < V; ++j) {
-      float f = to_f32(xv.v[j]) * sc + sh;
+      const float f = bn_pre(to_f32(xv.v[j]), sc, sh);
       yv.v[j] = from_f32<dev_t>(RELU ? fmaxf(f, 0.f) : f);
     }
     vstore<dev_t, V>(y + i, yv);
@@ -241,17 +245,19 @@
     Vec<dev_t, V> yv;
 #pragma unroll
     for (int j = 0; j < V; ++j) {
-      const float f = to_f32(xv.v[j]) * sc[j] + sh[j];
+      const float f = bn_pre(to_f32(xv.v[j]), sc[j], sh[j]);
       yv.v[j] = from_f32<dev_t>(RELU ? fmaxf(f, 0.f) : f);
     }
     vstore<dev_t, V>(y + r * C + c0, yv);
   }
 }
 
-template <typename dev_t, int V, bool RELU>
+template <typename dev_t, int V, bool RELU, bool MASK_Y = false>
 __global__ void bn_bwd_stats_nhwc_kernel(const dev_t* __restrict__ dy,
                                          const dev_t* __restrict__ x,
                                          const dev_t* __restrict__ y,
+                                         const float* __restrict__ scale,
+                                         const float* __restrict__ shift,
                                          const float* __restrict__ mean,
                                          const float* __restrict__ rstd,
                                          float* __restrict__ sums, int C,
@@ -264,11 +270,13 @@
   if (t < used) {
     const int c0 = (int)(t % lanes_per_row) * V;
     const int64_t rstride = used / lanes_per_row;
-    float mu[V], rs[V], s_dy[V], s_dyxh[V];
+    float mu[V], rs[V], sc[V], sh[V], s_dy[V], s_dyxh[V];
 #pragma unroll
     for (int j = 0; j < V; ++j) {
       mu[j] = mean[c0 + j];
       rs[j] = rstd[c0 + j];
+      sc[j] = (RELU && !MASK_Y) ? scale[c0 + j] : 0.f;
+      sh[j] = (RELU && !MASK_Y) ? shift[c0 + j] : 0.f;
       s_dy[j] = 0.f;
       s_dyxh[j] = 0.f;
     }
@@ -277,12 +285,14 @@
       Vec<dev_t, V> dyv = vload<dev_t, V>(dy + base);
       Vec<dev_t, V> xv = vload<dev_t, V>(x + base);
       Vec<dev_t, V> yv;
-      if (RELU) yv = vload<dev_t, V>(y + base);
+      if (RELU && MASK_Y) yv = vload<dev_t, V>(y + base);
 #pragma unroll
       for (int j = 0; j < V; ++j) {
         float g = to_f32(dyv.v[j]);
-        if (RELU && to_f32(yv.v[j]) <= 0.f) g = 0.f;
-        const float xh = (to_f32(xv.v[j]) - mu[j]) * rs[j];
+        const float xf = to_f32(xv.v[j]);
+        if (RELU && MASK_Y && to_f32(yv.v[j]) <= 0.f) g = 0.f;
+        if (RELU && !MASK_Y && !(bn_pre(xf, sc[j], sh[j]) > 0.f)) g = 0.f;
+        const float xh = (xf - mu[j]) * rs[j];
         s_dy[j] += g;
         s_dyxh[j] += g * xh;
       }
@@ -298,10 +308,12 @@
     atomicAdd(&sums[i], ls[i]);
 }
 
-template <typename dev_t, int V, bool RELU>
+template <typename dev_t, int V, bool RELU, bool MASK_Y = false>
 __global__ void bn_bwd_dx_nhwc_kernel(const dev_t* __restrict__ dy,
                                       const dev_t* __restrict__ x,
                                       const dev_t* __restrict__ y,
+                                      const float* __restrict__ scale,
+                                      const float* __restrict__ shift,
                                       const float* __restrict__ mean,
                                       const float* __restrict__ rstd,
                                       const float* __restrict__ weight,
@@ -314,12 +326,14 @@
   const int lanes_per_row = C / V;
   const int c0 = (int)(t % lanes_per_row) * V;
   const int64_t rstride = used / lanes_per_row;
-  float mu[V], rs[V], wr[V], m_dy[V], m_dyxh[V];
+  float mu[V], rs[V], wr[V], sc[V], sh[V], m_dy[V], m_dyxh[V];
 #pragma unroll
   for (int j = 0; j < V; ++j) {
     mu[j] = mean[c0 + j];
     rs[j] = rstd[c0 + j];
     wr[j] = weight[c0 + j] * rs[j];
+    sc[j] = (RELU && !MASK_Y) ? scale[c0 + j] : 0.f;
+    sh[j] = (RELU && !MASK_Y) ? shift[c0 + j] : 0.f;
     m_dy[j] = sums[c0 + j] * inv_count;
     m_dyxh[j] = sums[C + c0 + j] * inv_count;
   }
@@ -328,13 +342,15 @@
     Vec<dev_t, V> dyv = vload<dev_t, V>(dy + base);
     Vec<dev_t, V> xv = vload<dev_t, V>(x + base);
     Vec<dev_t, V> yv;
-    if (RELU) yv = vload<dev_t, V>(y + base);
+    if (RELU && MASK_Y) yv = vload<dev_t, V>(y + base);
     Vec<dev_t, V> dxv;
 #pragma unroll
     for (int j = 0; j < V; ++j) {
       float g = to_f32(dyv.v[j]);
-      if (RELU && to_f32(yv.v[j]) <= 0.f) g = 0.f;
-      const float xh = (to_f32(xv.v[j]) - mu[j]) * rs[j];
+      const float xf = to_f32(xv.v[j]);
+      if (RELU && MASK_Y && to_f32(yv.v[j]) <= 0.f) g = 0.f;
+      if (RELU && !MASK_Y && !(bn_pre(xf, sc[j], sh[j]) > 0.f)) g = 0.f;
+      const float xh = (xf - mu[j]) * rs[j];
       dxv.v[j] = from_f32<dev_t>(wr[j] * (g - m_dy[j] - xh * m_dyxh[j]));
     }
     vstore<dev_t, V>(dx + r * C + c0, dxv);
@@ -634,7 +650,7 @@
     }
   });
   HIP_CHECK_ERR();
-  return {y, mean, rstd};
+  return {y, mean, rstd, scale, shift};
 }
 
 std::vector<torch::Tensor> batchnorm_fwd_from_sums(
@@ -690,7 +706,7 @@
     }
   });
   HIP_CHECK_ERR();
-  return {y, mean, rstd};
+  return {y, mean, rstd, scale, shift};
 }
 
 torch::Tensor bn_apply(torch::Tensor x, torch::Tensor scale, torch::Tensor shift,
@@ -742,10 +758,13 @@
   return y;
 }
 
-std::vector<torch::Tensor> batchnorm_bwd(torch::Tensor dy, torch::Tensor x,
-                                         c10::optional<torch::Tensor> y,
-                                         torch::Tensor weight, torch::Tensor mean,
-                                         torch::Tensor rstd, bool relu) {
+bool bn_relu_mask_from_x(torch::Tensor x) { return dla::is_nhwc(x); }
+
+std::vector<torch::Tensor> batchnorm_bwd_ex(
+    torch::Tensor dy, torch::Tensor x, c10::optional<torch::Tensor> y,
+    torch::Tensor weight, torch::Tensor mean, torch::Tensor rstd,
+    c10::optional<torch::Tensor> scale, c10::optional<torch::Tensor> shift,
+    bool relu) {
   DLA_CHECK_CUDA(dy); DLA_CHECK_CUDA(x);
   const bool nhwc = dla::is_nhwc(x);
   TORCH_CHECK(nhwc || x.is_contiguous(), "batchnorm_bwd: x must be contiguous");
@@ -760,11 +779,32 @@
   auto w32 = weight.to(torch::kFloat);
   const int ysplit = (int)std::min<int64_t>((rows + 65535) / 65536 + 1,
                                             std::max(1, 2048 / C));
-  TORCH_CHECK(!relu || y.has_value(), "batchnorm_bwd: relu mask needs y");
+  const bool mask_y = relu && y.has_value();
+  if (relu && !mask_y) {
+    TORCH_CHECK(bn_relu_mask_from_x(x) && scale.has_value() && shift.has_value(),
+                "batchnorm_bwd: the relu mask needs y, or channels_last x "
+                "with the forward's scale and shift");
+    for (const auto* t : {&*scale, &*shift})
+      TORCH_CHECK(t->is_cuda() && t->scalar_type() == torch::kFloat &&
+                      t->is_contiguous() && t->numel() == C,
+                  "batchnorm_bwd: scale/shift must be contiguous fp32 [C]");
+  }
+  if (mask_y)
+    TORCH_CHECK(y->scalar_type() == x.scalar_type() && y->sizes() == x.sizes() &&
+                    (nhwc ? dla::is_nhwc(*y) : y->is_contiguous()),
+                "batchnorm_bwd: y must match x (shape, dtype, layout)");
+  const float* scp = (relu && !mask_y) ? scale->data_ptr<float>() : nullptr;
+  const float* shp = (relu && !mask_y) ? shift->data_ptr<float>() : nullptr;
   DLA_DISPATCH_FLOAT_TYPES(x.scalar_type(), "batchnorm_bwd", [&] {
-    const dev_t* yp = y.has_value() ? (const dev_t*)y->data_ptr() : nullptr;
-    auto launch_stats = [&](auto rtag) {
+    const dev_t* yp = mask_y ? (const dev_t*)y->data_ptr() : nullptr;
+    auto with_mode = [&](auto f) {
+      if (!relu) f(std::false_type{}, std::false_type{});
+      else if (mask_y) f(std::true_type{}, std::true_type{});
+      else f(std::true_type{}, std::false_type{});
+    };
+    with_mode([&](auto rtag, auto mtag) {
       constexpr bool R = decltype(rtag)::value;
+      constexpr bool MY = decltype(mtag)::value;
       if (nhwc) {
         constexpr int VM = 16 / (int)sizeof(dev_t);
         auto stats = [&](auto vtag) {
@@ -772,43 +812,46 @@
           const int lanes = C / V;
           const int64_t used = dla::nhwc_used_threads(lanes, rows, 262144);
           const int lds = 2 * C * sizeof(float);
-          hipLaunchKernelGGL((dla::bn_bwd_stats_nhwc_kernel<dev_t, V, R>),
+          hipLaunchKernelGGL((dla::bn_bwd_stats_nhwc_kernel<dev_t, V, R, MY>),
                              dim3((int)((used + 255) / 256)), dim3(256), lds,
                              dla::stream(), (const dev_t*)dy.data_ptr(),
-                             (const dev_t*)x.data_ptr(), yp, mean.data_ptr<float>(),
-                             rstd.data_ptr<float>(), sums.data_ptr<float>(), C,
-                             rows, used);
+                             (const dev_t*)x.data_ptr(), yp, scp, shp,
+                             mean.data_ptr<float>(), rstd.data_ptr<float>(),
+                             sums.data_ptr<float>(), C, rows, used);
         };
         if (C % VM == 0) stats(std::integral_constant<int, VM>{});
         else if (C % 2 == 0) stats(std::integral_constant<int, 2>{});
         else stats(std::integral_constant<int, 1>{});
-      } else {
+      } else if constexpr (!R || MY) {
         hipLaunchKernelGGL((dla::bn_bwd_stats_kernel<dev_t, R>), dim3(C, ysplit),
                            dim3(256), 0, dla::stream(), (const dev_t*)dy.data_ptr(),
                            (const dev_t*)x.data_ptr(), yp, mean.data_ptr<float>(),
                            rstd.data_ptr<float>(), sums.data_ptr<float>(), N, C, HW);
       }
-    };
-    if (relu) launch_stats(std::true_type{});
-    else launch_stats(std::false_type{});
+    });
 
     const int64_t n_total = x.numel();
     const float inv_count = 1.f / (float)rows;
     constexpr int VMAX = 16 / (int)sizeof(dev_t);
-    auto launch_dx = [&](auto vtag, auto rtag) {
-      constexpr int V = decltype(vtag)::value;
+    with_mode([&](auto rtag, auto mtag) {
       constexpr bool R = decltype(rtag)::value;
+      constexpr bool MY = decltype(mtag)::value;
       if (nhwc) {
-        const int lanes = C / V;
-        const int64_t used = dla::nhwc_used_threads(lanes, rows, 524288);
-        hipLaunchKernelGGL((dla::bn_bwd_dx_nhwc_kernel<dev_t, V, R>),
-                           dim3((int)((used + 255) / 256)), dim3(256), 0,
-                           dla::stream(), (const dev_t*)dy.data_ptr(),
-                           (const dev_t*)x.data_ptr(), yp, mean.data_ptr<float>(),
-                           rstd.data_ptr<float>(), w32.data_ptr<float>(),
-                           sums.data_ptr<float>(), (dev_t*)dx.data_ptr(), C,
-                           rows, used, inv_count);
-      } else {
+        auto dxk = [&](auto vtag) {
+          constexpr int V = decltype(vtag)::value;
+          const int lanes = C / V;
+          const int64_t used = dla::nhwc_used_threads(lanes, rows, 524288);
+          hipLaunchKernelGGL((dla::bn_bwd_dx_nhwc_kernel<dev_t, V, R, MY>),
+                             dim3((int)((used + 255) / 256)), dim3(256), 0,
+                             dla::stream(), (const dev_t*)dy.data_ptr(),
+                             (const dev_t*)x.data_ptr(), yp, scp, shp,
+                             mean.data_ptr<float>(), rstd.data_ptr<float>(),
+                             w32.data_ptr<float>(), sums.data_ptr<float>(),
+                             (dev_t*)dx.data_ptr(), C, rows, used, inv_count);
+        };
+        if (C % VMAX == 0) dxk(std::integral_constant<int, VMAX>{});
+        else dxk(std::integral_constant<int, 1>{});
+      } else if constexpr (!R || MY) {
         hipLaunchKernelGGL((dla::bn_bwd_dx_kernel<dev_t, R>), dim3(dla::grid_1d(n_total, 256)),
                            dim3(256), 0, dla::stream(), (const dev_t*)dy.data_ptr(),
                            (const dev_t*)x.data_ptr(), yp, mean.data_ptr<float>(),
@@ -816,19 +859,20 @@
                            sums.data_ptr<float>(), (dev_t*)dx.data_ptr(), C, HW,
                            n_total, inv_count);
       }
-    };
-    const bool vec_ok = nhwc && (C % VMAX == 0);
-    if (vec_ok) {
-      if (relu) launch_dx(std::integral_constant<int, VMAX>{}, std::true_type{});
-      else launch_dx(std::integral_constant<int, VMAX>{}, std::false_type{});
-    } else {
-      if (relu) launch_dx(std::integral_constant<int, 1>{}, std::true_type{});
-      else launch_dx(std::integral_constant<int, 1>{}, std::false_type{});
-    }
+    });
   });
   HIP_CHECK_ERR();
   return {dx, dla::bn_param_grad(sums, C, C, weight),
           dla::bn_param_grad(sums, 0, C, weight)};
+}
+
+std::vector<torch::Tensor> batchnorm_bwd(torch::Tensor dy, torch::Tensor x,
+                                         c10::optional<torch::Tensor> y,
+                                         torch::Tensor weight, torch::Tensor mean,
+                                         torch::Tensor rstd, bool relu) {
+  TORCH_CHECK(!relu || y.has_value(), "batchnorm_bwd: relu mask needs y");
+  return batchnorm_bwd_ex(dy, x, relu ? y : c10::nullopt, weight, mean, rstd,
+                          c10::nullopt, c10::nullopt, relu);
 }
 
 namespace dla {
@@ -945,7 +989,7 @@
     hipLaunchKernelGGL((dla::bn_bwd_dx_nhwc_kernel<dev_t, V, false>),
                        dim3((int)((used + 255) / 256)), dim3(256), 0,
                        dla::stream(), (const dev_t*)g.data_ptr(),
-                       (const dev_t*)x.data_ptr(), nullptr,
+                       (const dev_t*)x.data_ptr(), nullptr, nullptr, nullptr,
                        mean.data_ptr<float>(), rstd.data_ptr<float>(),
                        w32.data_ptr<float>(), sums.data_ptr<float>(),
                        (dev_t*)dx.data_ptr(), C, rows, used,
@@ -1010,3 +1054,296 @@
           dla::bn_param_grad(sums, 2 * C, C, weight_d),
           dbias.to(weight_d.scalar_type()).clone()};
 }
+
+namespace dla {
+
+constexpr int kPoolRun = 8;
+
+template <typename dev_t, int V>
+__global__ void __launch_bounds__(256)
+bn_relu_maxpool_fwd_nhwc_kernel(const dev_t* __restrict__ x,
+                                const float* __restrict__ scale,
+                                const float* __restrict__ shift,
+                                dev_t* __restrict__ out,
+                                uint8_t* __restrict__ slots, int C, int H,
+                                int W, int OH, int OW, int runs_per_img) {
+  const int n = blockIdx.x / runs_per_img;
+  const int oh0 = (blockIdx.x % runs_per_img) * kPoolRun;
+  const int oh1 = min(oh0 + kPoolRun, OH);
+  const int lanes = C / V;
+  const int items = (oh1 - oh0) * OW * lanes;
+  const dev_t* xn = x + (int64_t)n * H * W * C;
+  const int64_t obase = ((int64_t)n * OH + oh0) * OW * C;
+  for (int i = threadIdx.x; i < items; i += blockDim.x) {
+    const int c0 = (i % lanes) * V;
+    const int p = i / lanes;
+    const int ow = p % OW, oh = oh0 + p / OW;
+    float sc[V], sh[V], best[V];
+    int slot[V];
+#pragma unroll
+    for (int j = 0; j < V; ++j) {
+      sc[j] = scale[c0 + j];
+      sh[j] = shift[c0 + j];
+      best[j] = -INFINITY;
+      slot[j] = 4;
+    }
+#pragma unroll
+    for (int kh = 0; kh < 3; ++kh) {
+      const int ih = 2 * oh - 1 + kh;
+      if (ih < 0 || ih >= H) continue;
+#pragma unroll
+      for (int kw = 0; kw < 3; ++kw) {
+        const int iw = 2 * ow - 1 + kw;
+        if (iw < 0 || iw >= W) continue;
+        Vec<dev_t, V> xv =
+            vload<dev_t, V>(xn + ((int64_t)ih * W + iw) * C + c0);
+#pragma unroll
+        for (int j = 0; j < V; ++j) {
+          const float f = bn_pre(to_f32(xv.v[j]), sc[j], sh[j]);
+          const float y = to_f32(from_f32<dev_t>(fmaxf(f, 0.f)));
+          if (y > best[j]) {
+            best[j] = y;
+            slot[j] = kh * 3 + kw;
+          }
+        }
+      }
+    }
+    Vec<dev_t, V> ov;
+    Vec<uint8_t, V> sv;
+#pragma unroll
+    for (int j = 0; j < V; ++j) {
+      ov.v[j] = from_f32<dev_t>(best[j]);
+      sv.v[j] = (uint8_t)slot[j];
+    }
+    const int64_t o = obase + (int64_t)p * C + c0;
+    vstore<dev_t, V>(out + o, ov);
+    vstore<uint8_t, V>(slots + o, sv);
+  }
+}
+
+template <typename dev_t, int V>
+__device__ __forceinline__ void stem_pool_grad(
+    const dev_t* __restrict__ dpool, const uint8_t* __restrict__ slots,
+    const Vec<dev_t, V>& xv, const float* sc, const float* sh, int n, int h,
+    int w, int c0, int C, int OH, int OW, float* g) {
+#pragma unroll
+  for (int j = 0; j < V; ++j) g[j] = 0.f;
+  const int oh_hi = min((h + 1) >> 1, OH - 1);
+  const int ow_hi = min((w + 1) >> 1, OW - 1);
+  for (int oh = h >> 1; oh <= oh_hi; ++oh) {
+    const int kh = h - 2 * oh + 1;
+    for (int ow = w >> 1; ow <= ow_hi; ++ow) {
+      const int want = kh * 3 + (w - 2 * ow + 1);
+      const int64_t o = (((int64_t)n * OH + oh) * OW + ow) * C + c0;
+      Vec<uint8_t, V> sv = vload<uint8_t, V>(slots + o);
+      Vec<dev_t, V> dv = vload<dev_t, V>(dpool + o);
+#pragma unroll
+      for (int j = 0; j < V; ++j)
+        if ((int)sv.v[j] == want) g[j] += to_f32(dv.v[j]);
+    }
+  }
+#pragma unroll
+  for (int j = 0; j < V; ++j)
+    if (!(bn_pre(to_f32(xv.v[j]), sc[j], sh[j]) > 0.f)) g[j] = 0.f;
+}
+
+template <typename dev_t, int V>
+__global__ void bn_relu_maxpool_bwd_stats_nhwc_kernel(
+    const dev_t* __restrict__ dpool, const uint8_t* __restrict__ slots,
+    const dev_t* __restrict__ x, const float* __restrict__ scale,
+    const float* __restrict__ shift, const float* __restrict__ mean,
+    const float* __restrict__ rstd, float* __restrict__ sums, int C, int H,
+    int W, int OH, int OW, int64_t rows, int64_t used) {
+  extern __shared__ float ls[];
+  for (int i = threadIdx.x; i < 2 * C; i += blockDim.x) ls[i] = 0.f;
+  __syncthreads();
+  const int64_t t = (int64_t)blockIdx.x * blockDim.x + threadIdx.x;
+  const int lanes_per_row = C / V;
+  if (t < used) {
+    const int c0 = (int)(t % lanes_per_row) * V;
+    const int64_t rstride = used / lanes_per_row;
+    float mu[V], rs[V], sc[V], sh[V], s_g[V], s_gxh[V], g[V];
+#pragma unroll
+    for (int j = 0; j < V; ++j) {
+      mu[j] = mean[c0 + j];
+      rs[j] = rstd[c0 + j];
+      sc[j] = scale[c0 + j];
+      sh[j] = shift[c0 + j];
+      s_g[j] = 0.f;
+      s_gxh[j] = 0.f;
+    }
+    for (int64_t r = t / lanes_per_row; r < rows; r += rstride) {
+      const uint32_t r32 = (uint32_t)r;
+      const uint32_t q = r32 / (uint32_t)W;
+      const int w = (int)(r32 - q * (uint32_t)W);
+      const int n = (int)(q / (uint32_t)H);
+      const int h = (int)(q - (uint32_t)n * (uint32_t)H);
+      Vec<dev_t, V> xv = vload<dev_t, V>(x + r * C + c0);
+      stem_pool_grad<dev_t, V>(dpool, slots, xv, sc, sh, n, h, w, c0, C, OH,
+                               OW, g);
+#pragma unroll
+      for (int j = 0; j < V; ++j) {
+        const float xh = (to_f32(xv.v[j]) - mu[j]) * rs[j];
+        s_g[j] += g[j];
+        s_gxh[j] += g[j] * xh;
+      }
+    }
+#pragma unroll
+    for (int j = 0; j < V; ++j) {
+      atomicAdd(&ls[c0 + j], s_g[j]);
+      atomicAdd(&ls[C + c0 + j], s_gxh[j]);
+    }
+  }
+  __syncthreads();
+  for (int i = threadIdx.x; i < 2 * C; i += blockDim.x)
+    atomicAdd(&sums[i], ls[i]);
+}
+
+template <typename dev_t, int V>
+__global__ void bn_relu_maxpool_bwd_dx_nhwc_kernel(
+    const dev_t* __restrict__ dpool, const uint8_t* __restrict__ slots,
+    const dev_t* __restrict__ x, const float* __restrict__ scale,
+    const float* __restrict__ shift, const float* __restrict__ mean,
+    const float* __restrict__ rstd, const float* __restrict__ weight,
+    const float* __restrict__ sums, dev_t* __restrict__ dx, int C, int H,
+    int W, int OH, int OW, int64_t rows, int64_t used, float inv_count) {
+  const int64_t t = (int64_t)blockIdx.x * blockDim.x + threadIdx.x;
+  if (t >= used) return;
+  const int lanes_per_row = C / V;
+  const int c0 = (int)(t % lanes_per_row) * V;
+  const int64_t rstride = used / lanes_per_row;
+  float mu[V], rs[V], wr[V], sc[V], sh[V], m_g[V], m_gxh[V], g[V];
+#pragma unroll
+  for (int j = 0; j < V; ++j) {
+    mu[j] = mean[c0 + j];
+    rs[j] = rstd[c0 + j];
+    wr[j] = weight[c0 + j] * rs[j];
+    sc[j] = scale[c0 + j];
+    sh[j] = shift[c0 + j];
+    m_g[j] = sums[c0 + j] * inv_count;
+    m_gxh[j] = sums[C + c0 + j] * inv_count;
+  }
+  for (int64_t r = t / lanes_per_row; r < rows; r += rstride) {
+    const uint32_t r32 = (uint32_t)r;
+    const uint32_t q = r32 / (uint32_t)W;
+    const int w = (int)(r32 - q * (uint32_t)W);
+    const int n = (int)(q / (uint32_t)H);
+    const int h = (int)(q - (uint32_t)n * (uint32_t)H);
+    Vec<dev_t, V> xv = vload<dev_t, V>(x + r * C + c0);
+    stem_pool_grad<dev_t, V>(dpool, slots, xv, sc, sh, n, h, w, c0, C, OH, OW,
+                             g);
+    Vec<dev_t, V> dxv;
+#pragma unroll
+    for (int j = 0; j < V; ++j) {
+      const float xh = (to_f32(xv.v[j]) - mu[j]) * rs[j];
+      dxv.v[j] = from_f32<dev_t>(wr[j] * (g[j] - m_g[j] - xh * m_gxh[j]));
+    }
+    vstore<dev_t, V>(dx + r * C + c0, dxv);
+  }
+}
+
+inline void stem_check(const torch::Tensor& x, const char* fn) {
+  TORCH_CHECK(x.is_cuda() && x.dim() == 4 && is_nhwc_rows(x), fn,
+              ": x must be a channels_last 4D GPU tensor");
+  const int vmax = 16 / (int)x.element_size();
+  TORCH_CHECK(x.size(1) % vmax == 0, fn, ": C must be a multiple of ", vmax);
+  TORCH_CHECK(x.numel() > 0 && x.numel() / x.size(1) < (int64_t(1) << 31),
+              fn, ": N*H*W must be in [1, 2^31)");
+}
+
+}
+
+std::vector<torch::Tensor> bn_relu_maxpool_fwd(
+    torch::Tensor x, torch::Tensor weight, torch::Tensor bias,
+    c10::optional<torch::Tensor> running_mean,
+    c10::optional<torch::Tensor> running_var, double momentum, double eps) {
+  dla::stem_check(x, "bn_relu_maxpool_fwd");
+  const int N = (int)x.size(0), C = (int)x.size(1);
+  const int H = (int)x.size(2), W = (int)x.size(3);
+  const int OH = (H - 1) / 2 + 1, OW = (W - 1) / 2 + 1;
+  const int64_t rows = (int64_t)N * H * W;
+  auto sums = torch::zeros({2 * C}, x.options().dtype(torch::kFloat));
+  auto out_opts = x.options().memory_format(at::MemoryFormat::ChannelsLast);
+  auto pooled = torch::empty({N, C, OH, OW}, out_opts);
+  auto slots = torch::empty({N, C, OH, OW}, out_opts.dtype(torch::kByte));
+  const int runs = (OH + dla::kPoolRun - 1) / dla::kPoolRun;
+  TORCH_CHECK((int64_t)N * runs < (int64_t(1) << 31),
+              "bn_relu_maxpool_fwd: too many blocks");
+  dla::BnFinalized fin;
+  DLA_DISPATCH_FLOAT_TYPES(x.scalar_type(), "bn_relu_maxpool_fwd", [&] {
+    constexpr int V = 16 / (int)sizeof(dev_t);
+    const int64_t used = dla::nhwc_used_threads(C / V, rows, 262144);
+    hipLaunchKernelGGL((dla::bn_stats_nhwc_kernel<dev_t, V>),
+                       dim3((int)((used + 255) / 256)), dim3(256),
+                       2 * C * sizeof(float), dla::stream(),
+                       (const dev_t*)x.data_ptr(), sums.data_ptr<float>(), C,
+                       rows, used);
+    fin = dla::bn_finalize_launch(sums, weight, bias, running_mean,
+                                  running_var, C, rows, momentum, eps);
+    hipLaunchKernelGGL((dla::bn_relu_maxpool_fwd_nhwc_kernel<dev_t, V>),
+                       dim3(N * runs), dim3(256), 0, dla::stream(),
+                       (const dev_t*)x.data_ptr(), fin.scale.data_ptr<float>(),
+                       fin.shift.data_ptr<float>(), (dev_t*)pooled.data_ptr(),
+                       slots.data_ptr<uint8_t>(), C, H, W, OH, OW, runs);
+  });
+  HIP_CHECK_ERR();
+  return {pooled, slots, fin.mean, fin.rstd, fin.scale, fin.shift};
+}
+
+std::vector<torch::Tensor> bn_relu_maxpool_bwd(
+    torch::Tensor dpool, torch::Tensor x, torch::Tensor slots,
+    torch::Tensor weight, torch::Tensor mean, torch::Tensor rstd,
+    torch::Tensor scale, torch::Tensor shift) {
+  dla::stem_check(x, "bn_relu_maxpool_bwd");
+  const int N = (int)x.size(0), C = (int)x.size(1);
+  const int H = (int)x.size(2), W = (int)x.size(3);
+  const int OH = (H - 1) / 2 + 1, OW = (W - 1) / 2 + 1;
+  const int64_t rows = (int64_t)N * H * W;
+  DLA_CHECK_CUDA(dpool);
+  if (!dla::is_nhwc_rows(dpool))
+    dpool = dpool.contiguous(at::MemoryFormat::ChannelsLast);
+  const std::vector<int64_t> pshape{N, C, OH, OW};
+  TORCH_CHECK(dpool.scalar_type() == x.scalar_type() &&
+                  dpool.sizes() == at::IntArrayRef(pshape),
+              "bn_relu_maxpool_bwd: dpool must be [N, C, OH, OW] of x's dtype");
+  TORCH_CHECK(slots.is_cuda() && slots.scalar_type() == torch::kByte &&
+                  slots.sizes() == at::IntArrayRef(pshape) &&
+                  dla::is_nhwc_rows(slots),
+              "bn_relu_maxpool_bwd: slots must be channels_last uint8 "
+              "[N, C, OH, OW]");
+  for (const auto* t : {&mean, &rstd, &scale, &shift})
+    TORCH_CHECK(t->is_cuda() && t->scalar_type() == torch::kFloat &&
+                    t->is_contiguous() && t->numel() == C,
+                "bn_relu_maxpool_bwd: per-channel tensors must be contiguous "
+                "fp32 [C]");
+  TORCH_CHECK(weight.numel() == C, "bn_relu_maxpool_bwd: weight must be [C]");
+  auto sums = torch::zeros({2 * C}, x.options().dtype(torch::kFloat));
+  auto dx = torch::empty_like(x);
+  auto w32 = weight.to(torch::kFloat).contiguous();
+  DLA_DISPATCH_FLOAT_TYPES(x.scalar_type(), "bn_relu_maxpool_bwd", [&] {
+    constexpr int V = 16 / (int)sizeof(dev_t);
+    const int lanes = C / V;
+    const int64_t used_s = dla::nhwc_used_threads(lanes, rows, 262144);
+    hipLaunchKernelGGL((dla::bn_relu_maxpool_bwd_stats_nhwc_kernel<dev_t, V>),
+                       dim3((int)((used_s + 255) / 256)), dim3(256),
+                       2 * C * sizeof(float), dla::stream(),
+                       (const dev_t*)dpool.data_ptr(),
+                       slots.data_ptr<uint8_t>(), (const dev_t*)x.data_ptr(),
+                       scale.data_ptr<float>(), shift.data_ptr<float>(),
+                       mean.data_ptr<float>(), rstd.data_ptr<float>(),
+                       sums.data_ptr<float>(), C, H, W, OH, OW, rows, used_s);
+    const int64_t used = dla::nhwc_used_threads(lanes, rows, 524288);
+    hipLaunchKernelGGL((dla::bn_relu_maxpool_bwd_dx_nhwc_kernel<dev_t, V>),
+                       dim3((int)((used + 255) / 256)), dim3(256), 0,
+                       dla::stream(), (const dev_t*)dpool.data_ptr(),
+                       slots.data_ptr<uint8_t>(), (const dev_t*)x.data_ptr(),
+                       scale.data_ptr<float>(), shift.data_ptr<float>(),
+                       mean.data_ptr<float>(), rstd.data_ptr<float>(),
+                       w32.data_ptr<float>(), sums.data_ptr<float>(),
+                       (dev_t*)dx.data_ptr(), C, H, W, OH, OW, rows, used,
+                       1.f / (float)rows);
+  });
+  HIP_CHECK_ERR();
+  return {dx, dla::bn_param_grad(sums, C, C, weight),
+          dla::bn_param_grad(sums, 0, C, weight)};
+}
diff --git a/csrc/bindings.cpp b/csrc/bindings.cpp
--- a/csrc/bindings.cpp
+++ b/csrc/bindings.cpp
@@ -22,6 +22,20 @@
                                          c10::optional<torch::Tensor> y,
                                          torch::Tensor weight, torch::Tensor mean,
                                          torch::Tensor rstd, bool relu);
+bool bn_relu_mask_from_x(torch::Tensor x);
+std::vector<torch::Tensor> batchnorm_bwd_ex(
+    torch::Tensor dy, torch::Tensor x, c10::optional<torch::Tensor> y,
+    torch::Tensor weight, torch::Tensor mean, torch::Tensor rstd,
+    c10::optional<torch::Tensor> scale, c10::optional<torch::Tensor> shift,
+    bool relu);
+std::vector<torch::Tensor> bn_relu_maxpool_fwd(
+    torch::Tensor x, torch::Tensor weight, torch::Tensor bias,
+    c10::optional<torch::Tensor> running_mean,
+    c10::optional<torch::Tensor> running_var, double momentum, double eps);
+std::vector<torch::Tensor> bn_relu_maxpool_bwd(
+    torch::Tensor dpool, torch::Tensor x, torch::Tensor slots,
+    torch::Tensor weight, torch::Tensor mean, torch::Tensor rstd,
+    torch::Tensor scale, torch::Tensor shift);
 std::vector<torch::Tensor> batchnorm_fwd_from_sums(
     torch::Tensor x, torch::Tensor weight, torch::Tensor bias,
     torch::Tensor sums, c10::optional<torch::Tensor> running_mean,
@@ -128,6 +142,10 @@
   m.def("batchnorm_fwd_from_sums", &batchnorm_fwd_from_sums);
   m.def("bn_apply", &bn_apply);
   m.def("batchnorm_bwd", &batchnorm_bwd);
+  m.def("batchnorm_bwd_ex", &batchnorm_bwd_ex);
+  m.def("bn_relu_mask_from_x", &bn_relu_mask_from_x);
+  m.def("bn_relu_maxpool_fwd", &bn_relu_maxpool_fwd);
+  m.def("bn_relu_maxpool_bwd", &bn_relu_maxpool_bwd);
   m.def("bn_add_relu_fwd_from_sums", &bn_add_relu_fwd_from_sums);
   m.def("bn_add_relu_dual_fwd_from_sums", &bn_add_relu_dual_fwd_from_sums);
   m.def("bn_add_relu_bwd", &bn_add_relu_bwd);
diff --git a/deeplearning_amd/models/classification/resnet.py b/deeplearning_amd/models/classification/resnet.py
--- a/deeplearning_amd/models/classification/resnet.py
+++ b/deeplearning_amd/models/classification/resnet.py
@@ -3,7 +3,7 @@
 import torch
 import torch.nn as nn
 
-from ...ops import BatchNorm2d, add_relu
+from ...ops import BatchNorm2d, add_relu, bn_relu_maxpool
 from ...ops.conv1x1 import (can_pass_input, conv1x1_bn, conv_bn,
                             conv_bn_add_relu)
 from ..registry import register_model
@@ -156,7 +156,7 @@
         return nn.Sequential(*layers)
 
     def forward_features(self, x):
-        x = self.maxpool(self.bn1(self.conv1(x)))
+        x = bn_relu_maxpool(self.conv1(x), self.bn1, self.maxpool)
         x = self.layer1(x)
         x = self.layer2(x)
         x = self.layer3(x)
diff --git a/deeplearning_amd/ops/__init__.py b/deeplearning_amd/ops/__init__.py
--- a/deeplearning_amd/ops/__init__.py
+++ b/deeplearning_amd/ops/__init__.py
@@ -11,6 +11,7 @@
 from .losses import (CrossEntropyLoss, cross_entropy, sigmoid_focal_loss,
                      soft_target_cross_entropy)
 from .roi_align import MultiScaleRoIAlign, roi_align
+from .stem import bn_relu_maxpool, can_fuse_stem
 from .window import (roll_and_window_partition, window_merge_and_roll,
                      window_partition_eager, window_reverse_eager)
 
@@ -19,6 +20,7 @@
     "gelu", "silu", "add_relu", "GELU", "SiLU",
     "BatchNorm2d", "FrozenBatchNorm2d",
     "conv_bn", "conv1x1_bn", "conv_bn_add_relu",
+    "bn_relu_maxpool", "can_fuse_stem",
     "box_iou", "generalized_box_iou", "bbox_iou_aligned", "box_area", "nms",
     "batched_nms", "clip_boxes_to_image", "remove_small_boxes",
     "DropPath", "drop_path", "ModelEMA",
diff --git a/deeplearning_amd/ops/batchnorm.py b/deeplearning_amd/ops/batchnorm.py
--- a/deeplearning_amd/ops/batchnorm.py
+++ b/deeplearning_amd/ops/batchnorm.py
@@ -1,4 +1,6 @@
 from __future__ import annotations
+
+import os
 
 import torch
 import torch.nn as nn
@@ -7,21 +9,45 @@
 from ._ext import dense, ext, use_hip
 
 
+def _mask_from_y() -> bool:
+    return os.environ.get("DLA_BN_MASK_FROM_Y", "0") == "1"
+
+
+def save_bn_for_backward(ctx, x, y, weight, mean, rstd, scale, shift, relu):
+    ctx.relu = relu
+    ctx.mask_from_x = bool(relu and not _mask_from_y() and
+                           ext().bn_relu_mask_from_x(x))
+    if ctx.mask_from_x:
+        ctx.save_for_backward(x, weight, mean, rstd, scale, shift)
+    elif relu:
+        ctx.save_for_backward(x, weight, mean, rstd, y)
+    else:
+        ctx.save_for_backward(x, weight, mean, rstd)
+
+
+def bn_backward(ctx, dy):
+    x, weight, mean, rstd, *rest = ctx.saved_tensors
+    y = scale = shift = None
+    if ctx.mask_from_x:
+        scale, shift = rest
+    elif ctx.relu:
+        y, = rest
+    return ext().batchnorm_bwd_ex(dy, x, y, weight, mean, rstd, scale, shift,
+                                  ctx.relu)
+
+
 class _BNFn(torch.autograd.Function):
     @staticmethod
     def forward(ctx, x, weight, bias, running_mean, running_var, momentum, eps, relu):
         x = dense(x)
-        y, mean, rstd = ext().batchnorm_fwd(
+        y, mean, rstd, scale, shift = ext().batchnorm_fwd(
             x, weight, bias, running_mean, running_var, momentum, eps, relu)
-        ctx.save_for_backward(x, y, weight, mean, rstd)
-        ctx.relu = relu
+        save_bn_for_backward(ctx, x, y, weight, mean, rstd, scale, shift, relu)
         return y
 
     @staticmethod
     def backward(ctx, dy):
-        x, y, weight, mean, rstd = ctx.saved_tensors
-        dx, dw, db = ext().batchnorm_bwd(
-            dy, x, y if ctx.relu else None, weight, mean, rstd, ctx.relu)
+        dx, dw, db = bn_backward(ctx, dy)
         return dx, dw, db, None, None, None, None, None
 
 
diff --git a/deeplearning_amd/ops/conv1x1.py b/deeplearning_amd/ops/conv1x1.py
--- a/deeplearning_amd/ops/conv1x1.py
+++ b/deeplearning_amd/ops/conv1x1.py
@@ -7,6 +7,7 @@
 from torch import nn
 
 from ._ext import ext, use_hip
+from .batchnorm import bn_backward, save_bn_for_backward
 
 
 def _flatten_nhwc(x: torch.Tensor) -> torch.Tensor:
@@ -77,18 +78,16 @@
     @staticmethod
     def forward(ctx, x, weight, bias, sums, running_mean, running_var,
                 momentum, eps, relu):
-        y, mean, rstd = ext().batchnorm_fwd_from_sums(
+        y, mean, rstd, scale, shift = ext().batchnorm_fwd_from_sums(
             x, weight, bias, sums, running_mean, running_var, momentum, eps,
             relu)
-        ctx.save_for_backward(x, y, weight, mean, rstd)
-        ctx.relu = relu
+        save_bn_for_backward(ctx, x, y, weight, mean, rstd, scale, shift,
+                             relu)
         return y
 
     @staticmethod
     def backward(ctx, dy):
-        x, y, weight, mean, rstd = ctx.saved_tensors
-        dx, dw, db = ext().batchnorm_bwd(
-            dy, x, y if ctx.relu else None, weight, mean, rstd, ctx.relu)
+        dx, dw, db = bn_backward(ctx, dy)
         return dx, dw, db, None, None, None, None, None, None
 
 
diff --git a/deeplearning_amd/ops/stem.py b/deeplearning_amd/ops/stem.py
--- /dev/null
+++ b/deeplearning_amd/ops/stem.py
@@ -0,0 +1,69 @@
+from __future__ import annotations
+
+import os
+
+import torch
+from torch import nn
+
+from ._ext import ext, use_hip
+
+
+class _BNReluMaxPoolFn(torch.autograd.Function):
+    @staticmethod
+    def forward(ctx, x, weight, bias, running_mean, running_var, momentum,
+                eps):
+        pooled, slots, mean, rstd, scale, shift = ext().bn_relu_maxpool_fwd(
+            x, weight, bias, running_mean, running_var, momentum, eps)
+        ctx.save_for_backward(x, slots, weight, mean, rstd, scale, shift)
+        return pooled
+
+    @staticmethod
+    def backward(ctx, dpool):
+        x, slots, weight, mean, rstd, scale, shift = ctx.saved_tensors
+        dx, dw, db = ext().bn_relu_maxpool_bwd(dpool, x, slots, weight, mean,
+                                               rstd, scale, shift)
+        return dx, dw, db, None, None, None, None
+
+
+def _fused_stem_disabled() -> bool:
+    return os.environ.get("DLA_NO_FUSED_STEM", "0") == "1"
+
+
+def _pair(v):
+    return tuple(v) if isinstance(v, (tuple, list)) else (v, v)
+
+
+def can_fuse_stem(x: torch.Tensor, bn, pool) -> bool:
+    from .batchnorm import BatchNorm2d
+
+    if _fused_stem_disabled() or not use_hip(x):
+        return False
+    if type(bn) is not BatchNorm2d or not bn.relu or not bn.training:
+        return False
+    if type(pool) is not nn.MaxPool2d or pool.ceil_mode or \
+            pool.return_indices:
+        return False
+    if (_pair(pool.kernel_size), _pair(pool.stride), _pair(pool.padding),
+            _pair(pool.dilation)) != ((3, 3), (2, 2), (1, 1), (1, 1)):
+        return False
+    if x.dtype not in (torch.bfloat16, torch.float16, torch.float32):
+        return False
+    if x.dim() != 4 or x.numel() == 0 or \
+            x.shape[1] % (16 // x.element_size()) != 0:
+        return False
+    if x.shape[0] * x.shape[2] * x.shape[3] >= 2 ** 31:
+        return False
+    return x.is_contiguous(memory_format=torch.channels_last) and \
+        not x.is_contiguous()
+
+
+def bn_relu_maxpool(x: torch.Tensor, bn, pool) -> torch.Tensor:
+    if not can_fuse_stem(x, bn, pool):
+        return pool(bn(x))
+    if bn.running_mean.dtype != torch.float32:
+        bn.running_mean.data = bn.running_mean.data.float()
+        bn.running_var.data = bn.running_var.data.float()
+    if bn.num_batches_tracked is not None:
+        bn.num_batches_tracked.add_(1)
+    return _BNReluMaxPoolFn.apply(x, bn.weight, bn.bias, bn.running_mean,
+                                  bn.running_var, bn._eaf(), bn.eps)
```

Result: faster. 8391 images/s, median of 6 (+3.3%).
